# Oneaccount1/recommend-sys

Measured on NVIDIA B200. Metric: similarity_pairs_per_sec, higher is better.
Workload: dtype f64

## Files before the change

### recommend-sys_b200/csrc/api.cu

```cuda
#include <cstdlib>
#include <cstring>
#include <mutex>
#include <new>

#include "common.cuh"

static thread_local char g_err[512] = "";

void rs_set_error(const char *fmt, ...) {
    va_list ap;
    va_start(ap, fmt);
    vsnprintf(g_err, sizeof(g_err), fmt, ap);
    va_end(ap);
}

namespace {

int32_t enter(rs_knn *h) {
    if (!h) {
        rs_set_error("null handle");
        return RS_ERR_INVALID;
    }
    RS_CUDA(cudaSetDevice(h->device));
    return RS_OK;
}

struct Guard {
    std::unique_lock<std::recursive_mutex> lk;
    explicit Guard(rs_knn *h) { if (h) lk = std::unique_lock<std::recursive_mutex>(h->mu); }
};
#define RS_ENTER(h) Guard guard_(h); RS_TRY(enter(h))

void free_fit_state(rs_knn *h) {
    h->cur_chunk = 0;
    h->cur_off = 0;
    h->fitted = false;
    h->l_ptr = h->r_ptr = nullptr;
    h->l_col = h->r_col = nullptr;
    h->l_val = h->r_val = h->ld_val = nullptr;
    h->l_code = nullptr;
    h->means = h->stddevs = h->pmeans = h->left_bias = h->right_bias = nullptr;
    h->r_dev = nullptr;
    h->rd_col = nullptr;
    h->right_means = nullptr;
    h->cp = nullptr;
    h->l2r = nullptr;
    h->row_order = nullptr;
    h->row_heavy = nullptr;
    h->n_heavy = 0;
    h->n_pop = h->pop_ld = 0;
    h->pop_idx = h->pop_items = nullptr;
    h->pop_dense = nullptr;
    h->pop_blk = nullptr;
    h->w_ptr = nullptr;
    h->w_col = nullptr;
    h->w_dev = nullptr;
    h->row_all = nullptr;
    h->n_all_rows = 0;
    h->planes = nullptr;
    h->row_cnt = h->row_sum = nullptr;
    h->sims = nullptr;
    h->topk_idx = nullptr;
    h->topk_sim = nullptr;
    h->thr_key = nullptr;
    h->thr_id = nullptr;
    h->cand_cnt = nullptr;
    h->cand_id = nullptr;
    h->cand_sim = nullptr;
    h->row_flag = nullptr;
    h->d_flags = nullptr;
}

int32_t fold_profile(rs_knn *h) {
    RS_CUDA(cudaStreamSynchronize(h->stream));
    float ms = 0.f;
    if (h->prep_pending) {
        RS_CUDA(cudaEventElapsedTime(&ms, h->ev_a, h->ev_b));
        h->prof.prep_ms += ms;
        h->prep_pending = false;
    }
    if (h->sim_pending) {
        RS_CUDA(cudaEventElapsedTime(&ms, h->ev_b, h->ev_c));
        h->prof.sim_kernel_ms += ms;
        h->sim_pending = false;
    }
    if (h->pred_pending) {
        RS_CUDA(cudaEventElapsedTime(&ms, h->ev_d, h->ev_e));
        h->prof.predict_kernel_ms += ms;
        h->pred_pending = false;
    }
    return RS_OK;
}

bool tensor_eligible(const rs_knn *h) {
    if (h->rating_class != RS_CLASS_INT8) return false;
    if (h->p.sim == RS_SIM_COSINE || h->p.sim == RS_SIM_MSD || h->p.sim == RS_SIM_SLOPE_ONE) return true;
    if (h->p.sim == RS_SIM_PEARSON && h->p.pearson_mode == RS_PEARSON_SUMS) return true;
    return false;
}

bool tensor_faster(const rs_knn *h) {
    const double n = (double)h->n_left, rows = (double)(h->row_end - h->row_begin);
    const bool full = h->row_begin == 0 && h->row_end == h->n_left;
    const double g = h->p.sim == RS_SIM_COSINE ? 3.0 : h->p.sim == RS_SIM_MSD ? 4.0 : 6.0;
    const double pairs = full ? n * (n - 1.0) / 2.0 : rows * n;
    const double t_tensor = pairs * 2.0 * g * (double)h->n_right / 2.0e15 + 1e-4;
    const double triples = full ? h->triples : 2.0 * h->triples * (rows / n);
    const double t_stream = triples / 6.0e10 + 1e-4;
    return t_tensor <= t_stream;
}

struct IpcMap { int device; unsigned char handle[64]; void *base; };
std::mutex g_ipc_mu;
std::vector<IpcMap> g_ipc;

int32_t ipc_open_cached(int device, const unsigned char *hb, void **base) {
    std::lock_guard<std::mutex> lk(g_ipc_mu);
    for (const auto &m : g_ipc)
        if (m.device == device && !std::memcmp(m.handle, hb, 64)) { *base = m.base; return RS_OK; }
    cudaIpcMemHandle_t mh;
    std::memcpy(&mh, hb, 64);
    RS_CUDA(cudaIpcOpenMemHandle(base, mh, cudaIpcMemLazyEnablePeerAccess));
    IpcMap m;
    m.device = device;
    std::memcpy(m.handle, hb, 64);
    m.base = *base;
    g_ipc.push_back(m);
    return RS_OK;
}

int32_t init_handle(rs_knn *h) {
    RS_CUDA(cudaSetDevice(h->device));
    RS_CUDA(cudaStreamCreateWithFlags(&h->own_stream, cudaStreamNonBlocking));
    RS_CUDA(cudaStreamCreateWithFlags(&h->aux_stream, cudaStreamNonBlocking));
    RS_CUDA(cudaEventCreateWithFlags(&h->ev_in, cudaEventDisableTiming));
    RS_CUDA(cudaEventCreateWithFlags(&h->ev_fork, cudaEventDisableTiming));
    RS_CUDA(cudaEventCreateWithFlags(&h->ev_join, cudaEventDisableTiming));
    h->stream = h->own_stream;
    RS_CUDA(cudaEventCreate(&h->ev_a));
    RS_CUDA(cudaEventCreate(&h->ev_b));
    RS_CUDA(cudaEventCreate(&h->ev_c));
    RS_CUDA(cudaEventCreate(&h->ev_d));
    RS_CUDA(cudaEventCreate(&h->ev_e));
    return RS_OK;
}

}

extern "C" {

const char *rs_last_error(void) { return g_err; }
int32_t rs_knn_abi_version(void) { return 1; }

int32_t rs_knn_device_count(void) {
    int n = 0;
    if (cudaGetDeviceCount(&n) != cudaSuccess) {
        (void)cudaGetLastError();
        return 0;
    }
    return n;
}

int32_t rs_knn_params_default(rs_knn_params *p) {
    if (!p) return RS_ERR_INVALID;
    std::memset(p, 0, sizeof(*p));
    p->sim = RS_SIM_MSD;
    p->knn_type = RS_KNN_BASIC;
    p->k = 40;
    p->min_k = 1;
    p->device = -1;
    p->pearson_mode = RS_PEARSON_EXACT;
    p->sim_path = RS_PATH_AUTO;
    p->store = RS_STORE_MATRIX;
    p->topk = 40;
    return RS_OK;
}

int32_t rs_knn_create(const rs_knn_params *p, rs_knn **out) {
    if (!p || !out) {
        rs_set_error("rs_knn_create: null argument");
        return RS_ERR_INVALID;
    }
    if (p->sim < RS_SIM_COSINE || p->sim > RS_SIM_SLOPE_ONE || p->knn_type < RS_KNN_BASIC ||
        p->knn_type > RS_KNN_BASELINE || p->k < 1 || p->min_k < 0) {
        rs_set_error("rs_knn_create: invalid sim/knn_type/k/min_k");
        return RS_ERR_INVALID;
    }
    int ndev = 0;
    cudaError_t e = cudaGetDeviceCount(&ndev);
    if (e != cudaSuccess || ndev == 0) {
        (void)cudaGetLastError();
        rs_set_error("no CUDA device available (%s); this library has no CPU fallback",
                     e == cudaSuccess ? "0 devices" : cudaGetErrorString(e));
        return RS_ERR_CUDA;
    }
    int dev = p->device;
    if (dev < 0) RS_CUDA(cudaGetDevice(&dev));
    if (dev >= ndev) {
        rs_set_error("device %d out of range (%d devices)", dev, ndev);
        return RS_ERR_INVALID;
    }
    int cc_major = 0, cc_minor = 0;
    RS_CUDA(cudaDeviceGetAttribute(&cc_major, cudaDevAttrComputeCapabilityMajor, dev));
    RS_CUDA(cudaDeviceGetAttribute(&cc_minor, cudaDevAttrComputeCapabilityMinor, dev));
    if (cc_major != 10) {
        rs_set_error("device %d is sm_%d%d; this library is built for sm_100a (B200) only", dev, cc_major,
                     cc_minor);
        return RS_ERR_UNSUPPORTED;
    }
    rs_knn *h = new (std::nothrow) rs_knn();
    if (!h) return RS_ERR_OOM;
    h->p = *p;
    h->device = dev;
    const int32_t rc = init_handle(h);
    if (rc != RS_OK) {
        rs_knn_destroy(h);
        return rc;
    }
    *out = h;
    return RS_OK;
}

int32_t rs_knn_destroy(rs_knn *h) {
    if (!h) return RS_OK;
    cudaSetDevice(h->device);
    if (h->stream) cudaStreamSynchronize(h->stream);
    free_fit_state(h);
    for (auto &c : h->chunks) rs_cached_free(h->device, c.p, c.bytes);
    h->chunks.clear();
    if (h->tile_buf) cudaFree(h->tile_buf);
    if (h->band_buf) cudaFree(h->band_buf);
    if (h->ovf) rs_cached_free(h->device, h->ovf, h->ovf_bytes);
    for (size_t i = 0; i < h->scratch.size(); i++) rs_cached_free(h->device, h->scratch[i], h->scratch_bytes[i]);
    if (h->ev_a) cudaEventDestroy(h->ev_a);
    if (h->ev_b) cudaEventDestroy(h->ev_b);
    if (h->ev_c) cudaEventDestroy(h->ev_c);
    if (h->ev_d) cudaEventDestroy(h->ev_d);
    if (h->ev_e) cudaEventDestroy(h->ev_e);
    if (h->own_stream) cudaStreamDestroy(h->own_stream);
    if (h->aux_stream) cudaStreamDestroy(h->aux_stream);
    if (h->ev_in) cudaEventDestroy(h->ev_in);
    if (h->ev_fork) cudaEventDestroy(h->ev_fork);
    if (h->ev_join) cudaEventDestroy(h->ev_join);
    delete h;
    return RS_OK;
}

int32_t rs_knn_set_stream(rs_knn *h, void *cuda_stream, int32_t use_own) {
    RS_ENTER(h);
    RS_CUDA(cudaStreamSynchronize(h->stream));
    h->stream = use_own ? h->own_stream : reinterpret_cast<cudaStream_t>(cuda_stream);
    return RS_OK;
}

int32_t rs_knn_synchronize(rs_knn *h) {
    RS_ENTER(h);
    RS_CUDA(cudaStreamSynchronize(h->stream));
    return RS_OK;
}

int32_t rs_knn_fit_device(rs_knn *h, const int32_t *d_left, const int32_t *d_right, const double *d_rating,
                          int64_t nnz, int32_t n_left, int32_t n_right, double global_mean,
                          const double *d_left_bias, const double *d_right_bias, double global_bias) {
    RS_ENTER(h);
    if (!d_left || !d_right || !d_rating || nnz <= 0 || n_left <= 0 || n_right <= 0) {
        rs_set_error("rs_knn_fit: empty or null input (nnz=%lld n_left=%d n_right=%d)", (long long)nnz, n_left,
                     n_right);
        return RS_ERR_INVALID;
    }
    if (h->p.knn_type == RS_KNN_BASELINE && !d_left_bias) {
        rs_set_error("rs_knn_fit: RS_KNN_BASELINE needs left_bias (core/knn.go:179-187)");
        return RS_ERR_INVALID;
    }
    if (h->p.sim == RS_SIM_PEARSON_BASELINE && (!d_left_bias || !d_right_bias)) {
        rs_set_error("rs_knn_fit: RS_SIM_PEARSON_BASELINE needs both bias vectors");
        return RS_ERR_INVALID;
    }
    RS_TRY(fold_profile(h));
    free_fit_state(h);
    h->nnz = nnz;
    h->n_left = n_left;
    h->n_right = n_right;
    h->global_mean = global_mean;
    h->global_bias = global_bias;
    h->row_begin = h->p.row_begin;
    h->row_end = h->p.row_end;
    if (h->row_begin == 0 && h->row_end == 0) h->row_end = n_left;
    if (h->row_begin < 0 || h->row_end > n_left || h->row_begin > h->row_end) {
        rs_set_error("row shard [%lld,%lld) outside [0,%d)", (long long)h->row_begin, (long long)h->row_end, n_left);
        return RS_ERR_INVALID;
    }
    const int64_t rows = h->row_end - h->row_begin;
    if (h->p.shard_count < 0 || (h->p.shard_count >= 1 && (h->p.shard_index < 0 || h->p.shard_index >= h->p.shard_count))) {
        rs_set_error("shard_index %d outside [0, shard_count=%d)", h->p.shard_index, h->p.shard_count);
        return RS_ERR_INVALID;
    }
    if (h->p.shard_count >= 1 && rows != n_left) {
        rs_set_error("shard_count >= 1 and row_begin/row_end are two different sharding schemes: use one");
        return RS_ERR_INVALID;
    }
    h->cyc_R = (h->p.store == RS_STORE_MATRIX && h->p.shard_count >= 2) ? h->p.shard_count : 0;
    h->cyc_r = h->cyc_R ? h->p.shard_index : 0;
    h->peers_ready = false;
    if (h->cyc_R > RS_MAX_PEERS) {
        rs_set_error("at most %d cyclic row shards", RS_MAX_PEERS);
        return RS_ERR_UNSUPPORTED;
    }
    if (h->cyc_R && h->p.sim == RS_SIM_SLOPE_ONE) {
        rs_set_error("RS_SIM_SLOPE_ONE does not support cyclic row shards (use row_begin/row_end)");
        return RS_ERR_UNSUPPORTED;
    }
    h->rows_local = h->cyc_R ? rs_cyc_rows(n_left, h->cyc_R, h->cyc_r) : rows;

    RS_CUDA(cudaEventRecord(h->ev_a, h->stream));
    int32_t rc = rs_prep_build(h, d_left, d_right, d_rating, d_left_bias, d_right_bias);
    if (rc != RS_OK) { free_fit_state(h); return rc; }

    int path = h->p.sim_path;
    if (const char *force = getenv("RS_KNN_FORCE_PATH")) {
        if (!strcmp(force, "stream")) path = RS_PATH_STREAM;
        else if (!strcmp(force, "tensor")) path = RS_PATH_TENSOR;
    }
    if (h->p.sim == RS_SIM_SLOPE_ONE) {
        if (!tensor_eligible(h) || path == RS_PATH_STREAM) {
            rs_set_error("RS_SIM_SLOPE_ONE needs integer ratings in [-11,11] (tensor path)");
            free_fit_state(h);
            return RS_ERR_UNSUPPORTED;
        }
        path = RS_PATH_TENSOR;
    }
    if (h->cyc_R) {
        if (path == RS_PATH_TENSOR) {
            rs_set_error("cyclic row shards run the stream path; shard the tensor path with row_begin/row_end");
            free_fit_state(h);
            return RS_ERR_UNSUPPORTED;
        }
        path = RS_PATH_STREAM;
    }
    if (path == RS_PATH_AUTO) path = tensor_eligible(h) && tensor_faster(h) ? RS_PATH_TENSOR : RS_PATH_STREAM;
    if (path == RS_PATH_TENSOR && !tensor_eligible(h)) {
        rs_set_error("tensor path needs integer ratings in [-11,11] and Cosine/MSD (or Pearson in SUMS mode)");
        free_fit_state(h);
        return RS_ERR_UNSUPPORTED;
    }
    h->prof.sim_path_used = path;
    h->prof.corated_triples = h->triples;
    rc = (path == RS_PATH_TENSOR) ? rs_prep_planes(h) : rs_prep_rt(h);
    if (rc != RS_OK) { free_fit_state(h); return rc; }

    h->ld_s = ((int64_t)n_left + 15) / 16 * 16;
    if (h->p.store == RS_STORE_MATRIX) {
        rc = rs_alloc(h, &h->sims, (size_t)h->rows_local * (size_t)h->ld_s);
        if (rc != RS_OK) { free_fit_state(h); return rc; }
        RS_CUDA(cudaEventRecord(h->ev_b, h->stream));
        rc = (path == RS_PATH_TENSOR) ? rs_sim_tensor_launch(h, nullptr, 0, 0) : rs_sim_stream_launch(h);
        if (rc != RS_OK) { free_fit_state(h); return rc; }
        RS_CUDA(cudaEventRecord(h->ev_c, h->stream));
        if (path == RS_PATH_STREAM) {
            rc = rs_symmetrize_launch(h);
            if (rc != RS_OK) { free_fit_state(h); return rc; }
        }
    } else if (h->p.shard_count >= 1 && path == RS_PATH_TENSOR && rs_tensor_topk_fused(h)) {
        const int32_t k = h->p.topk > 0 ? h->p.topk : h->p.k;
        const int64_t n = n_left;
        h->cand_cap = 1792;
        if (const char *e = getenv("RS_KNN_TOPK_CAP")) h->cand_cap = atoi(e);
        if (k > 256 || h->cand_cap + k > 2048 || h->cand_cap < 1) {
            rs_set_error("fused top-k: k <= 256 and candidate capacity + k <= 2048 (k=%d cap=%d)", k, h->cand_cap);
            free_fit_state(h);
            return RS_ERR_UNSUPPORTED;
        }
        RS_TRY(rs_alloc(h, &h->topk_idx, (size_t)n * k));
        RS_TRY(rs_alloc(h, &h->topk_sim, (size_t)n * k));
        RS_TRY(rs_alloc(h, &h->thr_key, (size_t)n));
        RS_TRY(rs_alloc(h, &h->thr_id, (size_t)n));
        RS_TRY(rs_alloc(h, &h->cand_cnt, (size_t)n));
        RS_TRY(rs_alloc(h, &h->row_flag, (size_t)n));
        RS_TRY(rs_alloc(h, &h->cand_id, (size_t)n * h->cand_cap));
        RS_TRY(rs_alloc(h, &h->cand_sim, (size_t)n * h->cand_cap));
        h->topk_rows = n;
        RS_CUDA(cudaMemsetAsync(h->topk_idx, 0xFF, (size_t)n * k * 4, h->stream));
        RS_CUDA(cudaMemsetAsync(h->topk_sim, 0xFF, (size_t)n * k * 8, h->stream));
        RS_CUDA(cudaMemsetAsync(h->thr_key, 0, (size_t)n * 8, h->stream));
        RS_CUDA(cudaMemsetAsync(h->thr_id, 0xFF, (size_t)n * 4, h->stream));
        RS_CUDA(cudaMemsetAsync(h->cand_cnt, 0, (size_t)n * 4, h->stream));
        RS_CUDA(cudaMemsetAsync(h->row_flag, 0, (size_t)n * 4, h->stream));
        int32_t *d_over = h->d_flags + 14;
        RS_CUDA(cudaEventRecord(h->ev_b, h->stream));
        const int n_waves = rs_tensor_band_count(h);
        for (int w = 0; w < n_waves && rc == RS_OK; w++) {
            int rerun = 0;
            for (;;) {
                RS_CUDA(cudaMemsetAsync(d_over, 0, 4, h->stream));
                rc = rs_sim_tensor_band_launch(h, w);
                if (rc == RS_OK) rc = rs_topk_compact_launch(h, k, d_over, rerun);
                if (rc != RS_OK) break;
                int32_t over = 0;
                RS_CUDA(cudaMemcpyAsync(&over, d_over, 4, cudaMemcpyDeviceToHost, h->stream));
                RS_CUDA(cudaStreamSynchronize(h->stream));
                if (rerun) rc = rs_topk_mask_launch(h, k, 1);
                if (over == 0 || rc != RS_OK) break;
                rc = rs_topk_mask_launch(h, k, 0);
                rerun = 1;
            }
        }
        if (rc != RS_OK) { free_fit_state(h); return rc; }
        RS_CUDA(cudaEventRecord(h->ev_c, h->stream));
    } else if (h->p.shard_count >= 1) {
        const int32_t k = h->p.topk > 0 ? h->p.topk : h->p.k;
        const int64_t n = n_left;
        int64_t m = (int64_t)(6ll << 30) / (h->ld_s * 8);
        if (h->p.shard_count > 1) {
            int64_t want = (n + 4ll * h->p.shard_count - 1) / (4ll * h->p.shard_count);
            want = (want + 255) / 256 * 256;
            if (want < 1024) want = 1024;
            if (want < m) m = want;
        }
        if (const char *e = getenv("RS_KNN_SLAB_ROWS")) m = atoll(e);
        if (m < 256) m = 256;
        m = m / 256 * 256;
        if (m > n) m = (n + 15) / 16 * 16;
        const int64_t ld_t = m;
        double *tbuf = nullptr;
        RS_TRY(rs_alloc(h, &h->sims, (size_t)m * (size_t)h->ld_s));
        RS_TRY(rs_alloc(h, &tbuf, (size_t)n * (size_t)ld_t));
        RS_TRY(rs_alloc(h, &h->topk_idx, (size_t)n * k));
        RS_TRY(rs_alloc(h, &h->topk_sim, (size_t)n * k));
        h->topk_rows = n;
        RS_CUDA(cudaMemsetAsync(h->topk_idx, 0xFF, (size_t)n * k * 4, h->stream));
        RS_CUDA(cudaMemsetAsync(h->topk_sim, 0xFF, (size_t)n * k * 8, h->stream));
        RS_CUDA(cudaEventRecord(h->ev_b, h->stream));
        const int64_t n_slabs = (n + m - 1) / m;
        h->force_sym = true;
        for (int64_t sl = 0; sl < n_slabs; sl++) {
            const int64_t round = sl / h->p.shard_count, posn = sl % h->p.shard_count;
            const int64_t owner = (round & 1) ? h->p.shard_count - 1 - posn : posn;
            if (owner != h->p.shard_index) continue;
            const int64_t r0 = sl * m, r1 = r0 + m < n ? r0 + m : n;
            h->row_begin = r0;
            h->row_end = r1;
            h->col_begin = r0;
            if (path == RS_PATH_STREAM) {
                rc = cudaMemsetAsync(h->sims, 0xFF, (size_t)(r1 - r0) * (size_t)h->ld_s * 8, h->stream) == cudaSuccess
                         ? RS_OK : RS_ERR_CUDA;
                if (rc == RS_OK) rc = rs_sim_stream_launch(h);
            } else {
                rc = rs_sim_tensor_launch(h, nullptr, 0, 0);
            }
            if (rc == RS_OK) rc = rs_topk_slab_launch(h, r0, (int32_t)(r1 - r0), tbuf, ld_t, k);
            if (rc != RS_OK) break;
        }
        h->force_sym = false;
        h->col_begin = 0;
        h->row_begin = 0;
        h->row_end = n;
        if (rc != RS_OK) { free_fit_state(h); return rc; }
        RS_CUDA(cudaEventRecord(h->ev_c, h->stream));
    } else {
        const int32_t k = h->p.topk > 0 ? h->p.topk : h->p.k;
        int64_t slab = (int64_t)(2ull << 30) / ((int64_t)h->ld_s * 8);
        if (slab < 128) slab = 128;
        slab = slab / 128 * 128;
        if (slab > rows) slab = rows;
        RS_TRY(rs_alloc(h, &h->sims, (size_t)slab * (size_t)h->ld_s));
        RS_TRY(rs_alloc(h, &h->topk_idx, (size_t)rows * k));
        RS_TRY(rs_alloc(h, &h->topk_sim, (size_t)rows * k));
        h->topk_rows = rows;
        RS_CUDA(cudaEventRecord(h->ev_b, h->stream));
        const int64_t rb = h->row_begin, re = h->row_end;
        for (int64_t r0 = rb; r0 < re; r0 += slab) {
            h->row_begin = r0;
            h->row_end = r0 + slab < re ? r0 + slab : re;
            rc = (path == RS_PATH_TENSOR) ? rs_sim_tensor_launch(h, nullptr, 0, 0) : rs_sim_stream_launch(h);
            if (rc == RS_OK && path == RS_PATH_STREAM) rc = rs_symmetrize_launch(h);
            if (rc == RS_OK)
                rc = rs_topk_launch(h, k, h->topk_idx + (r0 - rb) * k, h->topk_sim + (r0 - rb) * k);
            if (rc != RS_OK) break;
        }
        h->row_begin = rb;
        h->row_end = re;
        if (rc != RS_OK) { free_fit_state(h); return rc; }
        RS_CUDA(cudaEventRecord(h->ev_c, h->stream));
    }
    h->prep_pending = true;
    h->sim_pending = true;
    h->fitted = true;
    return RS_OK;
}

int32_t rs_scratch_get(rs_knn *h, int slot, size_t bytes, void **out) {
    if (h->scratch.size() <= (size_t)slot) {
        h->scratch.resize(slot + 1, nullptr);
        h->scratch_bytes.resize(slot + 1, 0);
    }
    if (h->scratch_bytes[slot] < bytes) {
        if (h->scratch[slot]) {
            RS_CUDA(cudaStreamSynchronize(h->stream));
            rs_cached_free(h->device, h->scratch[slot], h->scratch_bytes[slot]);
        }
        h->scratch[slot] = nullptr;
        h->scratch_bytes[slot] = 0;
        size_t want = bytes + bytes / 4 + 256, got = 0;
        RS_TRY(rs_cached_malloc(h->device, &h->scratch[slot], want, &got));
        h->scratch_bytes[slot] = got;
    }
    *out = h->scratch[slot];
    return RS_OK;
}

int32_t rs_knn_fit(rs_knn *h, const int32_t *left, const int32_t *right, const double *rating, int64_t nnz,
                   int32_t n_left, int32_t n_right, double global_mean, const double *left_bias,
                   const double *right_bias, double global_bias) {
    RS_ENTER(h);
    if (!left || !right || !rating || nnz <= 0 || n_left <= 0 || n_right <= 0) {
        rs_set_error("rs_knn_fit: empty or null input (nnz=%lld n_left=%d n_right=%d)", (long long)nnz, n_left,
                     n_right);
        return RS_ERR_INVALID;
    }
    void *d_left, *d_right, *d_rating, *d_lb = nullptr, *d_rb = nullptr;
    RS_TRY(rs_scratch_get(h, 7, (size_t)nnz * 4, &d_left));
    RS_TRY(rs_scratch_get(h, 8, (size_t)nnz * 4, &d_right));
    RS_TRY(rs_scratch_get(h, 9, (size_t)nnz * 8, &d_rating));
    RS_CUDA(cudaMemcpyAsync(d_left, left, (size_t)nnz * 4, cudaMemcpyHostToDevice, h->stream));
    RS_CUDA(cudaMemcpyAsync(d_right, right, (size_t)nnz * 4, cudaMemcpyHostToDevice, h->stream));
    RS_CUDA(cudaMemcpyAsync(d_rating, rating, (size_t)nnz * 8, cudaMemcpyHostToDevice, h->stream));
    if (left_bias) {
        RS_TRY(rs_scratch_get(h, 10, (size_t)n_left * 8, &d_lb));
        RS_CUDA(cudaMemcpyAsync(d_lb, left_bias, (size_t)n_left * 8, cudaMemcpyHostToDevice, h->stream));
    }
    if (right_bias) {
        RS_TRY(rs_scratch_get(h, 11, (size_t)n_right * 8, &d_rb));
        RS_CUDA(cudaMemcpyAsync(d_rb, right_bias, (size_t)n_right * 8, cudaMemcpyHostToDevice, h->stream));
    }
    RS_CUDA(cudaEventRecord(h->ev_in, h->stream));
    RS_TRY(rs_knn_fit_device(h, (const int32_t *)d_left, (const int32_t *)d_right, (const double *)d_rating, nnz,
                             n_left, n_right, global_mean, (const double *)d_lb, (const double *)d_rb,
                             global_bias));
    cudaError_t e = cudaEventSynchronize(h->ev_in);
    if (e != cudaSuccess) {
        rs_set_error("rs_knn_fit: %s", cudaGetErrorString(e));
        h->fitted = false;
        return RS_ERR_CUDA;
    }
    return RS_OK;
}

static int32_t require_matrix(rs_knn *h, const char *who) {
    if (!h->fitted) {
        rs_set_error("%s: Fit has not been called", who);
        return RS_ERR_INVALID;
    }
    if (h->p.store != RS_STORE_MATRIX) {
        rs_set_error("%s needs RS_STORE_MATRIX (the handle keeps top-k lists only)", who);
        return RS_ERR_INVALID;
    }
    if (h->cyc_R > 1 && !h->peers_ready) {
        rs_set_error("%s: cyclic row shards hold one triangle of their rows until rs_knn_mirror has run", who);
        return RS_ERR_INVALID;
    }
    return RS_OK;
}

int32_t rs_knn_predict_batch_device(rs_knn *h, const int32_t *d_left, const int32_t *d_right, int64_t n,
                                    double *d_out) {
    RS_ENTER(h);
    RS_TRY(require_matrix(h, "rs_knn_predict_batch"));
    if (n == 0) return RS_OK;
    if (!d_left || !d_right || !d_out || n < 0) {
        rs_set_error("rs_knn_predict_batch: null argument");
        return RS_ERR_INVALID;
    }
    if (h->pred_pending) RS_TRY(fold_profile(h));
    RS_CUDA(cudaEventRecord(h->ev_d, h->stream));
    if (h->p.sim == RS_SIM_SLOPE_ONE) RS_TRY(rs_slope_predict_launch(h, d_left, d_right, n, d_out));
    else RS_TRY(rs_predict_launch(h, d_left, d_right, n, d_out, nullptr, nullptr, nullptr, 0));
    RS_CUDA(cudaEventRecord(h->ev_e, h->stream));
    h->pred_pending = true;
    return RS_OK;
}

int32_t rs_knn_predict_batch_sharded_device(rs_knn *h, const int32_t *d_left, const int32_t *d_right, int64_t n,
                                            double *d_out) {
    RS_ENTER(h);
    RS_TRY(require_matrix(h, "rs_knn_predict_batch_sharded"));
    if (h->cyc_R < 2) {
        rs_set_error("rs_knn_predict_batch_sharded: the handle is not a cyclic row shard");
        return RS_ERR_INVALID;
    }
    if (n == 0) return RS_OK;
    if (!d_left || !d_right || !d_out || n < 0) {
        rs_set_error("rs_knn_predict_batch_sharded: null argument");
        return RS_ERR_INVALID;
    }
    if (h->pred_pending) RS_TRY(fold_profile(h));
    RS_CUDA(cudaEventRecord(h->ev_d, h->stream));
    RS_TRY(rs_predict_launch(h, d_left, d_right, n, d_out, nullptr, nullptr, nullptr, 0, 1));
    RS_CUDA(cudaEventRecord(h->ev_e, h->stream));
    h->pred_pending = true;
    return RS_OK;
}

int32_t rs_knn_predict_batch(rs_knn *h, const int32_t *left, const int32_t *right, int64_t n, double *out) {
    RS_ENTER(h);
    RS_TRY(require_matrix(h, "rs_knn_predict_batch"));
    if (n == 0) return RS_OK;
    if (!left || !right || !out || n < 0) {
        rs_set_error("rs_knn_predict_batch: null argument");
        return RS_ERR_INVALID;
    }
    void *dl, *dr, *dout;
    RS_TRY(rs_scratch_get(h, 0, (size_t)n * 4, &dl));
    RS_TRY(rs_scratch_get(h, 1, (size_t)n * 4, &dr));
    RS_TRY(rs_scratch_get(h, 2, (size_t)n * 8, &dout));
    RS_CUDA(cudaMemcpyAsync(dl, left, (size_t)n * 4, cudaMemcpyHostToDevice, h->stream));
    RS_CUDA(cudaMemcpyAsync(dr, right, (size_t)n * 4, cudaMemcpyHostToDevice, h->stream));
    RS_TRY(rs_knn_predict_batch_device(h, (const int32_t *)dl, (const int32_t *)dr, n, (double *)dout));
    RS_CUDA(cudaMemcpyAsync(out, dout, (size_t)n * 8, cudaMemcpyDeviceToHost, h->stream));
    RS_CUDA(cudaStreamSynchronize(h->stream));
    return RS_OK;
}

int32_t rs_knn_predict_neighbors(rs_knn *h, int32_t left, int32_t right, int32_t cap, int32_t *ids, double *sims,
                                 int32_t *n_out) {
    RS_ENTER(h);
    RS_TRY(require_matrix(h, "rs_knn_predict_neighbors"));
    if (!ids || !sims || !n_out || cap < 1) {
        rs_set_error("rs_knn_predict_neighbors: null argument");
        return RS_ERR_INVALID;
    }
    void *dl, *dr, *dout, *dids, *dsims, *dcnt;
    RS_TRY(rs_scratch_get(h, 0, 4, &dl));
    RS_TRY(rs_scratch_get(h, 1, 4, &dr));
    RS_TRY(rs_scratch_get(h, 2, 8, &dout));
    RS_TRY(rs_scratch_get(h, 3, (size_t)cap * 4, &dids));
    RS_TRY(rs_scratch_get(h, 4, (size_t)cap * 8, &dsims));
    RS_TRY(rs_scratch_get(h, 5, 4, &dcnt));
    RS_CUDA(cudaMemcpyAsync(dl, &left, 4, cudaMemcpyHostToDevice, h->stream));
    RS_CUDA(cudaMemcpyAsync(dr, &right, 4, cudaMemcpyHostToDevice, h->stream));
    RS_CUDA(cudaMemsetAsync(dcnt, 0, 4, h->stream));
    RS_TRY(rs_predict_launch(h, (const int32_t *)dl, (const int32_t *)dr, 1, (double *)dout, (int32_t *)dids,
                             (double *)dsims, (int32_t *)dcnt, cap));
    RS_TRY(rs_nb_cells_launch(h, (const int32_t *)dl, (const int32_t *)dids, (const int32_t *)dcnt, (double *)dsims));
    int32_t cnt = 0;
    RS_CUDA(cudaMemcpyAsync(&cnt, dcnt, 4, cudaMemcpyDeviceToHost, h->stream));
    RS_CUDA(cudaStreamSynchronize(h->stream));
    if (cnt > 0) {
        RS_CUDA(cudaMemcpy(ids, dids, (size_t)cnt * 4, cudaMemcpyDeviceToHost));
        RS_CUDA(cudaMemcpy(sims, dsims, (size_t)cnt * 8, cudaMemcpyDeviceToHost));
    }
    *n_out = cnt;
    return RS_OK;
}

int32_t rs_knn_sims_rows(rs_knn *h, int64_t row0, int64_t nrows, double *out) {
    RS_ENTER(h);
    RS_TRY(require_matrix(h, "rs_knn_sims_rows"));
    if (!out || nrows < 0 || row0 < h->row_begin || row0 + nrows > h->row_end) {
        rs_set_error("rs_knn_sims_rows: rows [%lld,%lld) outside the shard [%lld,%lld)", (long long)row0,
                     (long long)(row0 + nrows), (long long)h->row_begin, (long long)h->row_end);
        return RS_ERR_INVALID;
    }
    if (nrows == 0) return RS_OK;
    int64_t local0 = row0 - h->row_begin;
    if (h->cyc_R > 1) {
        if (!rs_cyc_owns(row0, h->cyc_R, h->cyc_r) || row0 / RS_CYC_B != (row0 + nrows - 1) / RS_CYC_B) {
            rs_set_error("rs_knn_sims_rows: rows [%lld,%lld) are not inside one %d-row block of shard %d of %d",
                         (long long)row0, (long long)(row0 + nrows), RS_CYC_B, h->cyc_r, h->cyc_R);
            return RS_ERR_INVALID;
        }
        local0 = rs_cyc_local(row0, h->cyc_R);
    }
    RS_CUDA(cudaMemcpy2DAsync(out, (size_t)h->n_left * 8, h->sims + local0 * h->ld_s,
                              (size_t)h->ld_s * 8, (size_t)h->n_left * 8, (size_t)nrows, cudaMemcpyDeviceToHost,
                              h->stream));
    RS_CUDA(cudaStreamSynchronize(h->stream));
    return RS_OK;
}

int32_t rs_knn_topk_device(rs_knn *h, int32_t k, int32_t *d_idx, double *d_sim) {
    RS_ENTER(h);
    if (!h->fitted || !d_idx || !d_sim) {
        rs_set_error("rs_knn_topk: not fitted or null argument");
        return RS_ERR_INVALID;
    }
    const int64_t rows = h->p.store == RS_STORE_TOPK ? h->topk_rows : h->rows_local;
    if (h->p.store == RS_STORE_MATRIX) RS_TRY(require_matrix(h, "rs_knn_topk"));
    if (h->p.store == RS_STORE_TOPK) {
        const int32_t kk = h->p.topk > 0 ? h->p.topk : h->p.k;
        if (k != kk) {
            rs_set_error("rs_knn_topk: handle holds top-%d lists, asked for %d", kk, k);
            return RS_ERR_INVALID;
        }
        RS_CUDA(cudaMemcpyAsync(d_idx, h->topk_idx, (size_t)rows * k * 4, cudaMemcpyDeviceToDevice, h->stream));
        RS_CUDA(cudaMemcpyAsync(d_sim, h->topk_sim, (size_t)rows * k * 8, cudaMemcpyDeviceToDevice, h->stream));
        return RS_OK;
    }
    return rs_topk_launch(h, k, d_idx, d_sim);
}

int32_t rs_knn_topk(rs_knn *h, int32_t k, int32_t *idx, double *sim) {
    RS_ENTER(h);
    if (!h->fitted || !idx || !sim || k < 1) {
        rs_set_error("rs_knn_topk: not fitted or bad argument");
        return RS_ERR_INVALID;
    }
    const int64_t rows = h->p.store == RS_STORE_TOPK ? h->topk_rows : h->rows_local;
    void *di, *ds;
    RS_TRY(rs_scratch_get(h, 3, (size_t)rows * k * 4, &di));
    RS_TRY(rs_scratch_get(h, 4, (size_t)rows * k * 8, &ds));
    RS_TRY(rs_knn_topk_device(h, k, (int32_t *)di, (double *)ds));
    RS_CUDA(cudaMemcpyAsync(idx, di, (size_t)rows * k * 4, cudaMemcpyDeviceToHost, h->stream));
    RS_CUDA(cudaMemcpyAsync(sim, ds, (size_t)rows * k * 8, cudaMemcpyDeviceToHost, h->stream));
    RS_CUDA(cudaStreamSynchronize(h->stream));
    return RS_OK;
}

int32_t rs_knn_cosums(rs_knn *h, int64_t row0, int64_t nrows, int32_t *out) {
    RS_ENTER(h);
    if (!h->fitted || !out || nrows < 0 || row0 < 0 || row0 + nrows > h->n_left) {
        rs_set_error("rs_knn_cosums: not fitted or bad argument");
        return RS_ERR_INVALID;
    }
    if (h->rating_class != RS_CLASS_INT8) {
        rs_set_error("rs_knn_cosums: integer co-rating sums need integer ratings in [-11,11]");
        return RS_ERR_UNSUPPORTED;
    }
    if (nrows == 0) return RS_OK;
    if (!h->planes) RS_TRY(rs_prep_planes(h));
    void *d;
    const size_t bytes = (size_t)nrows * (size_t)h->n_left * 6 * 4;
    RS_TRY(rs_scratch_get(h, 6, bytes, &d));
    RS_TRY(rs_sim_tensor_launch(h, (int32_t *)d, row0, nrows));
    RS_CUDA(cudaMemcpyAsync(out, d, bytes, cudaMemcpyDeviceToHost, h->stream));
    RS_CUDA(cudaStreamSynchronize(h->stream));
    return RS_OK;
}

static int32_t copy_vec(rs_knn *h, const double *d, double *out, const char *who) {
    RS_ENTER(h);
    if (!h->fitted || !out || !d) {
        rs_set_error("%s: not fitted or null argument", who);
        return RS_ERR_INVALID;
    }
    RS_CUDA(cudaMemcpyAsync(out, d, (size_t)h->n_left * 8, cudaMemcpyDeviceToHost, h->aux_stream));
    RS_CUDA(cudaStreamSynchronize(h->aux_stream));
    return RS_OK;
}

int32_t rs_knn_means(rs_knn *h, double *out) { return copy_vec(h, h ? h->means : nullptr, out, "rs_knn_means"); }
int32_t rs_knn_stddevs(rs_knn *h, double *out) {
    if (h && h->p.knn_type != RS_KNN_ZSCORE) {
        rs_set_error("rs_knn_stddevs: only the z-score KNN keeps StdDevs (core/knn.go:167)");
        return RS_ERR_INVALID;
    }
    return copy_vec(h, h ? h->stddevs : nullptr, out, "rs_knn_stddevs");
}

int32_t rs_knn_set_k(rs_knn *h, int32_t k, int32_t min_k) {
    RS_ENTER(h);
    if (k < 1 || min_k < 0) {
        rs_set_error("rs_knn_set_k: k >= 1 and min_k >= 0 required");
        return RS_ERR_INVALID;
    }
    h->p.k = k;
    h->p.min_k = min_k;
    return RS_OK;
}

int32_t rs_knn_peer_export(rs_knn *h, unsigned char *handle64, int64_t *offset) {
    RS_ENTER(h);
    if (!h->fitted || h->cyc_R < 2 || !handle64 || !offset) {
        rs_set_error("rs_knn_peer_export: the handle is not a fitted cyclic row shard");
        return RS_ERR_INVALID;
    }
    for (const auto &c : h->chunks) {
        const char *s0 = reinterpret_cast<const char *>(h->sims);
        if (s0 >= c.p && s0 < c.p + c.bytes) {
            cudaIpcMemHandle_t mh;
            RS_CUDA(cudaIpcGetMemHandle(&mh, c.p));
            static_assert(sizeof(mh) == 64, "cudaIpcMemHandle_t is 64 bytes");
            std::memcpy(handle64, &mh, 64);
            *offset = (int64_t)(s0 - c.p);
            return RS_OK;
        }
    }
    rs_set_error("rs_knn_peer_export: the matrix is not in the handle's arena");
    return RS_ERR_INVALID;
}

int32_t rs_knn_peer_import(rs_knn *h, int32_t n_peers, const unsigned char *handles, const int64_t *offsets) {
    RS_ENTER(h);
    if (!h->fitted || h->cyc_R < 2 || n_peers != h->cyc_R || !handles || !offsets) {
        rs_set_error("rs_knn_peer_import: needs a fitted cyclic row shard and one (handle, offset) per shard");
        return RS_ERR_INVALID;
    }
    for (int q = 0; q < n_peers; q++) {
        if (q == h->cyc_r) { h->peer_sims[q] = h->sims; continue; }
        const unsigned char *hb = handles + (size_t)q * 64;
        void *base = nullptr;
        RS_TRY(ipc_open_cached(h->device, hb, &base));
        h->peer_sims[q] = reinterpret_cast<const double *>(static_cast<const char *>(base) + offsets[q]);
    }
    return RS_OK;
}

int32_t rs_knn_peer_import_local(rs_knn *h, int32_t n_peers, rs_knn *const *peers) {
    RS_ENTER(h);
    if (!h->fitted || h->cyc_R < 2 || n_peers != h->cyc_R || !peers) {
        rs_set_error("rs_knn_peer_import_local: needs a fitted cyclic row shard and one handle per shard");
        return RS_ERR_INVALID;
    }
    for (int q = 0; q < n_peers; q++) {
        const rs_knn *o = peers[q];
        if (!o || !o->fitted || o->cyc_R != h->cyc_R || o->cyc_r != q || o->n_left != h->n_left || o->ld_s != h->ld_s) {
            rs_set_error("rs_knn_peer_import_local: peer %d is not shard %d of the same Fit", q, q);
            return RS_ERR_INVALID;
        }
        if (o->device != h->device) {
            int can = 0;
            RS_CUDA(cudaDeviceCanAccessPeer(&can, h->device, o->device));
            if (!can) {
                rs_set_error("device %d cannot access device %d", h->device, o->device);
                return RS_ERR_UNSUPPORTED;
            }
            cudaError_t e = cudaDeviceEnablePeerAccess(o->device, 0);
            if (e != cudaSuccess && e != cudaErrorPeerAccessAlreadyEnabled) RS_CUDA(e);
            (void)cudaGetLastError();
        }
        h->peer_sims[q] = o->sims;
    }
    return RS_OK;
}

int32_t rs_knn_mirror(rs_knn *h) {
    RS_ENTER(h);
    if (!h->fitted || h->cyc_R < 2) {
        rs_set_error("rs_knn_mirror: the handle is not a fitted cyclic row shard");
        return RS_ERR_INVALID;
    }
    for (int q = 0; q < h->cyc_R; q++)
        if (q != h->cyc_r && !h->peer_sims[q]) {
            rs_set_error("rs_knn_mirror: shard %d has not been attached (rs_knn_peer_import)", q);
            return RS_ERR_INVALID;
        }
    RS_TRY(rs_mirror_launch(h));
    h->peers_ready = true;
    return RS_OK;
}

int32_t rs_knn_profile_get(rs_knn *h, rs_knn_profile *out) {
    RS_ENTER(h);
    if (!out) return RS_ERR_INVALID;
    RS_TRY(fold_profile(h));
    *out = h->prof;
    return RS_OK;
}

namespace {
struct HostBlock { void *p; size_t bytes; bool used; };
std::mutex g_host_mu;
std::vector<HostBlock> g_host;
}

int32_t rs_knn_host_alloc(size_t bytes, void **out) {
    if (!out) { rs_set_error("rs_knn_host_alloc: null argument"); return RS_ERR_INVALID; }
    if (bytes == 0) bytes = 1;
    std::lock_guard<std::mutex> lk(g_host_mu);
    HostBlock *best = nullptr;
    for (auto &b : g_host)
        if (!b.used && b.bytes >= bytes && b.bytes <= 2 * bytes + 4096 && (!best || b.bytes < best->bytes)) best = &b;
    if (best) { best->used = true; *out = best->p; return RS_OK; }
    void *p = nullptr;
    RS_CUDA(cudaHostAlloc(&p, bytes, cudaHostAllocPortable));
    g_host.push_back({p, bytes, true});
    *out = p;
    return RS_OK;
}

int32_t rs_knn_host_free(void *p) {
    if (!p) return RS_OK;
    std::lock_guard<std::mutex> lk(g_host_mu);
    for (auto &b : g_host)
        if (b.p == p && b.used) { b.used = false; return RS_OK; }
    rs_set_error("rs_knn_host_free: not a block of rs_knn_host_alloc");
    return RS_ERR_INVALID;
}

int32_t rs_knn_trim_cache(void) {
    rs_cache_trim();
    {
        std::lock_guard<std::mutex> lk(g_host_mu);
        size_t kept = 0;
        for (auto &b : g_host) {
            if (b.used) g_host[kept++] = b;
            else cudaFreeHost(b.p);
        }
        g_host.resize(kept);
    }
    std::lock_guard<std::mutex> lk(g_ipc_mu);
    int cur = 0;
    cudaGetDevice(&cur);
    for (const auto &m : g_ipc) {
        cudaSetDevice(m.device);
        cudaIpcCloseMemHandle(m.base);
    }
    g_ipc.clear();
    cudaSetDevice(cur);
    return RS_OK;
}

int32_t rs_knn_profile_reset(rs_knn *h) {
    RS_ENTER(h);
    RS_TRY(fold_profile(h));
    int32_t path = h->prof.sim_path_used;
    h->prof = rs_knn_profile{};
    h->prof.sim_path_used = path;
    h->prof.corated_triples = h->triples;
    return RS_OK;
}

}
```

### recommend-sys_b200/csrc/common.cuh

```cuda
#pragma once

#include <cuda_runtime.h>

#include <cstdarg>
#include <cstdint>
#include <cstdio>
#include <mutex>
#include <vector>

#include "rs_knn.h"

void rs_set_error(const char *fmt, ...);

#define RS_CUDA(expr)                                                                       \
    do {                                                                                    \
        cudaError_t e_ = (expr);                                                            \
        if (e_ != cudaSuccess) {                                                            \
            rs_set_error("%s: %s (%s:%d)", #expr, cudaGetErrorString(e_), __FILE__, __LINE__); \
            return (e_ == cudaErrorMemoryAllocation) ? RS_ERR_OOM : RS_ERR_CUDA;            \
        }                                                                                   \
    } while (0)

#define RS_TRY(expr)              \
    do {                          \
        int32_t rc_ = (expr);     \
        if (rc_ != RS_OK) return rc_; \
    } while (0)

enum { RS_CLASS_INT8 = 0, RS_CLASS_TABLE = 1 };
constexpr int RS_INT8_BIAS = 12;

constexpr int RS_STREAM_WARPS = 8;

constexpr int RS_TC_BM = 128;
constexpr int RS_TC_BN = 64;
constexpr int RS_TC_BK = 128;
constexpr int RS_TC_KBLK = 256;

constexpr int RS_CYC_B = 32;
constexpr int RS_MAX_PEERS = 16;
__host__ __device__ inline int64_t rs_cyc_local(int64_t i, int count) {
    return (i / ((int64_t)RS_CYC_B * count)) * RS_CYC_B + i % RS_CYC_B;
}
__host__ __device__ inline bool rs_cyc_owns(int64_t i, int count, int index) {
    return (i / RS_CYC_B) % count == index;
}
inline int64_t rs_cyc_rows(int64_t n, int count, int index) {
    const int64_t nblk = (n + RS_CYC_B - 1) / RS_CYC_B;
    int64_t rows = 0;
    for (int64_t b = index; b < nblk; b += count) rows += (b + 1) * RS_CYC_B <= n ? RS_CYC_B : n - b * RS_CYC_B;
    return rows;
}

struct rs_knn {
    std::recursive_mutex mu;
    rs_knn_params p{};
    int device = 0;
    cudaStream_t own_stream = nullptr;
    cudaStream_t stream = nullptr;
    cudaStream_t aux_stream = nullptr;
    cudaEvent_t ev_in = nullptr;
    cudaEvent_t ev_fork = nullptr, ev_join = nullptr;
    cudaEvent_t ev_a = nullptr, ev_b = nullptr, ev_c = nullptr, ev_d = nullptr, ev_e = nullptr;
    rs_knn_profile prof{};
    bool sim_pending = false, pred_pending = false, prep_pending = false;

    bool fitted = false;
    int32_t n_left = 0, n_right = 0;
    int64_t nnz = 0;
    int64_t row_begin = 0, row_end = 0;
    int64_t col_begin = 0;
    bool force_sym = false;
    int64_t topk_rows = 0;
    int32_t cyc_R = 0, cyc_r = 0;
    int64_t rows_local = 0;
    int64_t n_work_rows = 0;
    const double *peer_sims[RS_MAX_PEERS] = {nullptr};
    bool peers_ready = false;
    double global_mean = 0.0, global_bias = 0.0;
    int rating_class = RS_CLASS_INT8;

    struct Chunk { char *p; size_t bytes; };
    std::vector<Chunk> chunks;
    size_t cur_chunk = 0, cur_off = 0;
    void *tile_buf = nullptr;
    size_t tile_buf_bytes = 0;
    int64_t tile_key[5] = {-1, -1, -1, -1, -1};
    int32_t tile_count = 0;
    void *band_buf = nullptr;
    size_t band_buf_bytes = 0;
    int64_t band_key[4] = {-1, -1, -1, -1};
    std::vector<int64_t> band_off;
    unsigned long long *thr_key = nullptr;
    int32_t *thr_id = nullptr;
    int32_t *cand_cnt = nullptr;
    int32_t *cand_id = nullptr;
    double *cand_sim = nullptr;
    int32_t cand_cap = 0;
    int32_t *row_flag = nullptr;

    int64_t *l_ptr = nullptr;
    int32_t *l_col = nullptr;
    double *l_val = nullptr;
    uint8_t *l_code = nullptr;
    double *ld_val = nullptr;
    int64_t *r_ptr = nullptr;
    int32_t *r_col = nullptr;
    double *r_val = nullptr;

    double *means = nullptr;
    double *stddevs = nullptr;
    double *pmeans = nullptr;
    double *left_bias = nullptr;
    int32_t *row_cnt = nullptr;
    int32_t *row_sum = nullptr;
    int64_t max_row_cnt = 0;
    int32_t max_right_len = 0;
    double triples = 0.0;
    double *right_bias = nullptr;
    int32_t *rd_col = nullptr;
    double *right_means = nullptr;

    double *r_dev = nullptr;
    int32_t *cp = nullptr;
    int32_t n_chunks = 0;
    int32_t stream_jc = 256;
    bool stream_lower = false;
    double inc_upper = 0.0, inc_lower = 0.0;
    int64_t *l2r = nullptr;
    int32_t *perm_lr = nullptr, *perm_rl = nullptr, *perm_tmp = nullptr;
    int32_t *row_order = nullptr;
    int32_t *row_heavy = nullptr;
    int32_t n_heavy = 0;
    int32_t n_pop = 0, pop_ld = 0;
    bool pop_u8 = false;
    int32_t *pop_idx = nullptr;
    int32_t *pop_items = nullptr;
    uint8_t *pop_blk = nullptr;
    void *pop_dense = nullptr;
    int64_t *w_ptr = nullptr;
    int32_t *w_col = nullptr;
    double *w_dev = nullptr;
    int32_t *row_all = nullptr;
    int64_t n_all_rows = 0;
    int8_t *planes = nullptr;
    int64_t tc_npad = 0, tc_kpad = 0;

    double *sims = nullptr;
    int64_t ld_s = 0;
    int32_t *topk_idx = nullptr;
    double *topk_sim = nullptr;

    int32_t *d_flags = nullptr;
    void *ovf = nullptr;
    size_t ovf_bytes = 0;
    std::vector<void *> scratch;
    std::vector<size_t> scratch_bytes;
};

int32_t rs_cached_malloc(int device, void **out, size_t bytes, size_t *got);
void rs_cached_free(int device, void *p, size_t bytes);
void rs_cache_trim(void);

extern "C" int32_t rs_scratch_get(rs_knn *h, int slot, size_t bytes, void **out);

int32_t rs_prep_build(rs_knn *h, const int32_t *d_left, const int32_t *d_right, const double *d_rating,
                      const double *d_left_bias, const double *d_right_bias);
int32_t rs_dev_alloc(rs_knn *h, void **out, size_t bytes);
template <typename T>
inline int32_t rs_alloc(rs_knn *h, T **out, size_t count) {
    return rs_dev_alloc(h, reinterpret_cast<void **>(out), count * sizeof(T));
}
int32_t rs_prep_rt(rs_knn *h);
int32_t rs_prep_planes(rs_knn *h);

int32_t rs_sim_stream_launch(rs_knn *h);
int32_t rs_symmetrize_launch(rs_knn *h);
int32_t rs_mirror_launch(rs_knn *h);

int32_t rs_sim_tensor_launch(rs_knn *h, int32_t *d_cosums, int64_t cos_row0, int64_t cos_nrows);
int32_t rs_tensor_band_count(const rs_knn *h);
int32_t rs_sim_tensor_band_launch(rs_knn *h, int32_t wave);
bool rs_tensor_topk_fused(const rs_knn *h);

int32_t rs_predict_launch(rs_knn *h, const int32_t *d_left, const int32_t *d_right, int64_t n, double *d_out,
                          int32_t *d_nb_ids, double *d_nb_sims, int32_t *d_nb_count, int32_t nb_cap, int32_t foreign_zero = 0);
int32_t rs_nb_cells_launch(rs_knn *h, const int32_t *d_left, const int32_t *d_nb_ids, const int32_t *d_nb_count,
                           double *d_nb_sims);
int32_t rs_topk_launch(rs_knn *h, int32_t k, int32_t *d_idx, double *d_sim);
int32_t rs_slope_predict_launch(rs_knn *h, const int32_t *d_left, const int32_t *d_right, int64_t n, double *d_out);
int32_t rs_topk_slab_launch(rs_knn *h, int64_t g0, int32_t m, double *tbuf, int64_t ld_t, int32_t k);
int32_t rs_topk_compact_launch(rs_knn *h, int32_t k, int32_t *d_overflow, int rerun);
int32_t rs_topk_mask_launch(rs_knn *h, int32_t k, int restore);

__host__ __device__ inline uint64_t rs_sim_key(double s) {
    s = s + 0.0;
#ifdef __CUDA_ARCH__
    uint64_t b = (uint64_t)__double_as_longlong(s);
#else
    uint64_t b;
    __builtin_memcpy(&b, &s, 8);
#endif
    return (b & 0x8000000000000000ull) ? ~b : (b | 0x8000000000000000ull);
}
__host__ __device__ inline double rs_key_sim(uint64_t k) {
    uint64_t b = (k & 0x8000000000000000ull) ? (k & 0x7fffffffffffffffull) : ~k;
#ifdef __CUDA_ARCH__
    return __longlong_as_double((long long)b);
#else
    double s;
    __builtin_memcpy(&s, &b, 8);
    return s;
#endif
}
```

### recommend-sys_b200/csrc/prep.cu

```cuda
#include <cub/cub.cuh>

#include <cstdlib>
#include <cstring>

#include "common.cuh"

int32_t rs_dev_alloc(rs_knn *h, void **out, size_t bytes) {
    bytes = (bytes + 255) & ~(size_t)255;
    if (bytes == 0) bytes = 256;
    while (h->cur_chunk < h->chunks.size()) {
        rs_knn::Chunk &c = h->chunks[h->cur_chunk];
        if (h->cur_off + bytes <= c.bytes) {
            *out = c.p + h->cur_off;
            h->cur_off += bytes;
            return RS_OK;
        }
        h->cur_chunk++;
        h->cur_off = 0;
    }
    const size_t min_chunk = (size_t)64 << 20;
    const size_t want = bytes > min_chunk ? bytes : min_chunk;
    void *p = nullptr;
    size_t got = 0;
    RS_TRY(rs_cached_malloc(h->device, &p, want, &got));
    h->chunks.push_back({(char *)p, got});
    h->cur_chunk = h->chunks.size() - 1;
    h->cur_off = bytes;
    *out = p;
    return RS_OK;
}

namespace {

constexpr int T = 256;
inline unsigned blocks_for(int64_t n, int t = T) { return (unsigned)((n + t - 1) / t); }

enum { FLAG_BAD_ID = 1, FLAG_NOT_INT8 = 2, FLAG_DUP = 4, FLAG_NAN = 8 };

__global__ void iota_validate_kernel(const int32_t *__restrict__ left, const int32_t *__restrict__ right,
                                     const double *__restrict__ rating, int64_t nnz, int32_t n_left,
                                     int32_t n_right, int32_t *__restrict__ idx, int32_t *__restrict__ flags) {
    int64_t i = (int64_t)blockIdx.x * blockDim.x + threadIdx.x;
    if (i >= nnz) return;
    idx[i] = (int32_t)i;
    int32_t l = left[i], r = right[i];
    int f = 0;
    if (l < 0 || l >= n_left || r < 0 || r >= n_right) f |= FLAG_BAD_ID;
    double v = rating[i];
    if (v != v) f |= FLAG_NAN;
    if (!(v == rint(v) && fabs(v) <= 11.0)) f |= FLAG_NOT_INT8;
    if (f) atomicOr(flags, f);
}

__global__ void ptr_from_sorted_kernel(const int32_t *__restrict__ keys, int64_t nnz, int32_t n_rows,
                                       int64_t *__restrict__ ptr) {
    const int64_t i = (int64_t)blockIdx.x * blockDim.x + threadIdx.x;
    if (i > nnz) return;
    const int32_t cur = i < nnz ? keys[i] : n_rows;
    const int32_t prev = i > 0 ? keys[i - 1] : -1;
    for (int32_t k = prev + 1; k <= cur; k++) ptr[k] = i;
}

__global__ void gather_keys_kernel(const int32_t *__restrict__ src, const int32_t *__restrict__ perm, int64_t n,
                                   int32_t *__restrict__ out) {
    int64_t i = (int64_t)blockIdx.x * blockDim.x + threadIdx.x;
    if (i < n) out[i] = src[perm[i]];
}

__global__ void gather_csr_kernel(const int32_t *__restrict__ perm, const int32_t *__restrict__ minor,
                                  const double *__restrict__ rating, int64_t nnz, int32_t *__restrict__ col,
                                  double *__restrict__ val) {
    int64_t i = (int64_t)blockIdx.x * blockDim.x + threadIdx.x;
    if (i >= nnz) return;
    int32_t p = perm[i];
    col[i] = minor[p];
    val[i] = rating[p];
}

__global__ void dup_check_kernel(const int32_t *__restrict__ row, const int32_t *__restrict__ col, int64_t nnz,
                                 int32_t *__restrict__ flags) {
    int64_t i = (int64_t)blockIdx.x * blockDim.x + threadIdx.x;
    if (i == 0 || i >= nnz) return;
    if (row[i] == row[i - 1] && col[i] == col[i - 1]) atomicOr(flags, FLAG_DUP);
}

__global__ void gather_val_kernel(const int32_t *__restrict__ perm, const double *__restrict__ rating, int64_t nnz,
                                  double *__restrict__ val) {
    int64_t i = (int64_t)blockIdx.x * blockDim.x + threadIdx.x;
    if (i < nnz) val[i] = rating[perm[i]];
}

__global__ void code_int8_kernel(const double *__restrict__ val, int64_t nnz, uint8_t *__restrict__ code) {
    int64_t i = (int64_t)blockIdx.x * blockDim.x + threadIdx.x;
    if (i < nnz) code[i] = (uint8_t)((int)val[i] + RS_INT8_BIAS);
}

__global__ void row_isum_kernel(const int64_t *__restrict__ l_ptr, const uint8_t *__restrict__ l_code,
                                int32_t n_left, int32_t *__restrict__ row_cnt, int32_t *__restrict__ row_sum) {
    int32_t row = (int32_t)(((int64_t)blockIdx.x * blockDim.x + threadIdx.x) >> 5);
    int lane = threadIdx.x & 31;
    if (row >= n_left) return;
    int s = 0;
    for (int64_t x = l_ptr[row] + lane; x < l_ptr[row + 1]; x += 32) s += (int)l_code[x] - RS_INT8_BIAS;
    for (int o = 16; o > 0; o >>= 1) s += __shfl_xor_sync(0xffffffffu, s, o);
    if (lane == 0) {
        row_cnt[row] = (int32_t)(l_ptr[row + 1] - l_ptr[row]);
        row_sum[row] = s;
    }
}

__device__ __forceinline__ double ordered_sum(const double *__restrict__ v, int64_t b, int64_t e, int lane,
                                              double mean, bool squared_dev) {
    double sum = 0.0;
    for (int64_t base = b; base < e; base += 32) {
        double x = (base + lane < e) ? v[base + lane] : 0.0;
        if (squared_dev) x = (x - mean) * (x - mean);
        const int lim = (e - base) < 32 ? (int)(e - base) : 32;
        for (int q = 0; q < lim; q++) sum += __shfl_sync(0xffffffffu, x, q);
    }
    return sum;
}

__global__ void row_stats_ordered_kernel(const int64_t *__restrict__ l_ptr, const double *__restrict__ ld_val,
                                         const double *__restrict__ l_val, int32_t n_left, int want_mean,
                                         int want_std, double *__restrict__ means, double *__restrict__ stddevs,
                                         double *__restrict__ pmeans) {
    const int32_t i = (int32_t)(((int64_t)blockIdx.x * blockDim.x + threadIdx.x) >> 5);
    const int lane = threadIdx.x & 31;
    if (i >= n_left) return;
    const int64_t b = l_ptr[i], e = l_ptr[i + 1];
    const double count = (double)(e - b);
    double mean = means[i];
    if (want_mean) {
        mean = ordered_sum(ld_val, b, e, lane, 0.0, false) / count;
        const double pm = ordered_sum(l_val, b, e, lane, 0.0, false) / count;
        if (lane == 0) { means[i] = mean; pmeans[i] = pm; }
    }
    if (want_std) {
        const double s2 = ordered_sum(ld_val, b, e, lane, mean, true);
        if (lane == 0) stddevs[i] = sqrt(s2 / count) + 1e-5;
    }
}

__global__ void means_from_isum_kernel(const int32_t *__restrict__ row_cnt, const int32_t *__restrict__ row_sum,
                                       int32_t n_left, double *__restrict__ means, double *__restrict__ pmeans) {
    const int32_t i = blockIdx.x * blockDim.x + threadIdx.x;
    if (i >= n_left) return;
    const double m = (double)row_sum[i] / (double)row_cnt[i];
    means[i] = m;
    pmeans[i] = m;
}

__global__ void build_rdev_kernel(const int64_t *__restrict__ r_ptr, const int32_t *__restrict__ r_col,
                                  const double *__restrict__ r_val, int32_t n_right, int sim,
                                  const double *__restrict__ pmeans, const double *__restrict__ left_bias,
                                  const double *__restrict__ right_bias, double global_bias,
                                  double *__restrict__ r_dev) {
    const int32_t c = (int32_t)(((int64_t)blockIdx.x * blockDim.x + threadIdx.x) >> 5);
    const int lane = threadIdx.x & 31;
    if (c >= n_right) return;
    for (int64_t x = r_ptr[c] + lane; x < r_ptr[c + 1]; x += 32) {
        const int32_t j = r_col[x];
        const double y = r_val[x];
        double t;
        if (sim == RS_SIM_PEARSON) t = y - pmeans[j];
        else if (sim == RS_SIM_PEARSON_BASELINE) { const double base = global_bias + left_bias[j]; const double bb = base + right_bias[c]; t = y - bb; }
        else t = y;
        r_dev[x] = t;
    }
}

__global__ void row_len_kernel(const int64_t *__restrict__ l_ptr, int32_t n_left, int32_t *__restrict__ len,
                               int32_t *__restrict__ ids) {
    const int32_t i = blockIdx.x * blockDim.x + threadIdx.x;
    if (i >= n_left) return;
    len[i] = (int32_t)(l_ptr[i + 1] - l_ptr[i]);
    ids[i] = i;
}

__global__ void build_cp_kernel(const int64_t *__restrict__ r_ptr, const int32_t *__restrict__ r_col,
                                int32_t n_right, int32_t q0, int32_t n_q, int32_t jc, int32_t *__restrict__ cp) {
    const int32_t c = (int32_t)(((int64_t)blockIdx.x * blockDim.x + threadIdx.x) >> 5);
    const int lane = threadIdx.x & 31;
    if (c >= n_right) return;
    const int64_t b = r_ptr[c], e = r_ptr[c + 1];
    int32_t *out = cp + (int64_t)c * (n_q + 1);
    auto rel = [&](int32_t col) {
        const int32_t q = col / jc - q0;
        return q < 0 ? -1 : (q >= n_q ? n_q : q);
    };
    for (int64_t x0 = b; x0 <= e; x0 += 32) {
        const int64_t x = x0 + lane;
        if (x > e) continue;
        const int32_t cur = x < e ? rel(r_col[x]) : n_q;
        const int32_t prev = x > b ? rel(r_col[x - 1]) : -1;
        for (int32_t q = prev + 1; q <= cur; q++) out[q] = (int32_t)(x - b);
    }
}

__global__ void invert_perm_kernel(const int32_t *__restrict__ perm, int64_t n, int32_t *__restrict__ inv) {
    const int64_t x = (int64_t)blockIdx.x * blockDim.x + threadIdx.x;
    if (x < n) inv[perm[x]] = (int32_t)x;
}
__global__ void compose_l2r_kernel(const int32_t *__restrict__ perm_lr, const int32_t *__restrict__ inv_rl, int64_t n,
                                   int64_t *__restrict__ l2r) {
    const int64_t e = (int64_t)blockIdx.x * blockDim.x + threadIdx.x;
    if (e < n) l2r[e] = inv_rl[perm_lr[e]];
}

__global__ void pop_count_kernel(const int32_t *__restrict__ len_sorted, int32_t n, int64_t min_len, int32_t cap,
                                 int32_t *__restrict__ out) {
    int32_t lo = 0, hi = n;
    while (lo < hi) {
        const int32_t mid = (lo + hi) >> 1;
        if ((int64_t)len_sorted[mid] >= min_len) lo = mid + 1; else hi = mid;
    }
    *out = lo < cap ? lo : cap;
}
__global__ void pop_index_kernel(const int32_t *__restrict__ sorted, int32_t n_pop, int32_t pop_ld,
                                 int32_t *__restrict__ pop_idx, int32_t *__restrict__ pop_items,
                                 uint8_t *__restrict__ pop_blk) {
    const int32_t p = blockIdx.x * blockDim.x + threadIdx.x;
    if (p >= pop_ld) return;
    if (p < n_pop) { const int32_t i = sorted[p]; pop_idx[i] = p; pop_items[p] = i; pop_blk[i >> 5] = 1; }
    else pop_items[p] = -1;
}
template <typename DT>
__global__ void pop_scatter_kernel(const int64_t *__restrict__ r_ptr, const int32_t *__restrict__ r_col,
                                   const double *__restrict__ r_val, const double *__restrict__ r_dev,
                                   int32_t n_right, const int32_t *__restrict__ pop_idx, int32_t pop_ld,
                                   DT *__restrict__ dense, int64_t *__restrict__ w_cnt) {
    const int32_t c = (int32_t)(((int64_t)blockIdx.x * blockDim.x + threadIdx.x) >> 5);
    const int lane = threadIdx.x & 31;
    if (c > n_right) return;
    if (c == n_right) { if (lane == 0) w_cnt[c] = 0; return; }
    int32_t light = 0;
    for (int64_t x = r_ptr[c] + lane; x < r_ptr[c + 1]; x += 32) {
        const int32_t p = pop_idx[r_col[x]];
        if (p < 0) { light++; continue; }
        if (sizeof(DT) == 1) dense[(int64_t)c * pop_ld + p] = (DT)((int)r_val[x] + RS_INT8_BIAS);
        else dense[(int64_t)c * pop_ld + p] = (DT)r_dev[x];
    }
#pragma unroll
    for (int o = 16; o > 0; o >>= 1) light += __shfl_xor_sync(0xffffffffu, light, o);
    if (lane == 0) w_cnt[c] = light;
}
__global__ void pop_compact_kernel(const int64_t *__restrict__ r_ptr, const int32_t *__restrict__ r_col,
                                   const double *__restrict__ r_dev, int32_t n_right,
                                   const int32_t *__restrict__ pop_idx, const int64_t *__restrict__ w_ptr,
                                   int32_t *__restrict__ w_col, double *__restrict__ w_dev, int64_t *__restrict__ pos) {
    const int32_t c = (int32_t)(((int64_t)blockIdx.x * blockDim.x + threadIdx.x) >> 5);
    const int lane = threadIdx.x & 31;
    if (c >= n_right) return;
    const int64_t b = r_ptr[c], e = r_ptr[c + 1];
    int64_t out = w_ptr[c];
    for (int64_t x0 = b; x0 < e; x0 += 32) {
        const int64_t x = x0 + lane;
        int32_t j = -1;
        bool keep = false;
        if (x < e) { j = r_col[x]; keep = pop_idx[j] < 0; }
        const unsigned m = __ballot_sync(0xffffffffu, keep);
        if (x < e) {
            const int64_t o = out + __popc(m & ((1u << lane) - 1u));
            if (keep) { w_col[o] = j; w_dev[o] = r_dev[x]; pos[x] = o; }
            else pos[x] = -1;
        }
        out += __popc(m);
    }
}
__global__ void pop_remap_l2r_kernel(int64_t *__restrict__ l2r, const int64_t *__restrict__ pos, int64_t n) {
    const int64_t e = (int64_t)blockIdx.x * blockDim.x + threadIdx.x;
    if (e < n) l2r[e] = pos[l2r[e]];
}
struct PopLight {
    const int32_t *pop_idx;
    __host__ __device__ bool operator()(const int32_t &i) const { return pop_idx[i] < 0; }
};


__global__ void scatter_planes_kernel(const int64_t *__restrict__ l_ptr, const int32_t *__restrict__ l_col,
                                      const uint8_t *__restrict__ l_code, int32_t n_left, int64_t npad,
                                      int64_t kpad, int32_t kblk, int8_t *__restrict__ planes) {
    int32_t row = (int32_t)(((int64_t)blockIdx.x * blockDim.x + threadIdx.x) >> 5);
    int lane = threadIdx.x & 31;
    if (row >= n_left) return;
    int64_t plane = npad * kpad;
    for (int64_t x = l_ptr[row] + lane; x < l_ptr[row + 1]; x += 32) {
        int v = (int)l_code[x] - RS_INT8_BIAS;
        const int32_t col = l_col[x];
        int64_t o = ((int64_t)(col / kblk) * npad + row) * kblk + (col % kblk);
        planes[o] = (int8_t)(v * v);
        planes[plane + o] = 1;
        planes[2 * plane + o] = (int8_t)v;
    }
}

struct CycOwned {
    int count, index;
    __host__ __device__ bool operator()(const int32_t &i) const { return rs_cyc_owns(i, count, index); }
};

struct SortTmp {
    void *p = nullptr;
    size_t bytes = 0;
};

int bits_for(int32_t n) {
    int b = 1;
    while ((1ll << b) < (long long)n) b++;
    return b;
}

}

#define RS_SORT_PAIRS(keys_in, keys_out, vals_in, vals_out, n, end_bit)                                      \
    do {                                                                                                     \
        size_t need_ = 0;                                                                                    \
        RS_CUDA(cub::DeviceRadixSort::SortPairs(nullptr, need_, keys_in, keys_out, vals_in, vals_out, (int)(n), \
                                                0, end_bit, st));                                            \
        if (need_ > tmp.bytes) {                                                                             \
            RS_TRY(rs_dev_alloc(h, &tmp.p, need_));                                                          \
            tmp.bytes = need_;                                                                               \
        }                                                                                                    \
        RS_CUDA(cub::DeviceRadixSort::SortPairs(tmp.p, tmp.bytes, keys_in, keys_out, vals_in, vals_out,      \
                                                (int)(n), 0, end_bit, st));                                  \
    } while (0)

__global__ void triples_kernel(const int64_t *__restrict__ r_ptr, int32_t nr, unsigned long long *out,
                               int32_t *max_len) {
    unsigned long long acc = 0;
    int32_t mx = 0;
    for (int64_t c = blockIdx.x * (int64_t)blockDim.x + threadIdx.x; c < nr; c += (int64_t)gridDim.x * blockDim.x) {
        const int32_t cnt = (int32_t)(r_ptr[c + 1] - r_ptr[c]);
        const unsigned long long n = (unsigned long long)cnt;
        acc += n * (n - (n ? 1 : 0)) / 2;
        mx = cnt > mx ? cnt : mx;
    }
#pragma unroll
    for (int o = 16; o > 0; o >>= 1) { const int32_t v = __shfl_xor_sync(0xffffffffu, mx, o); mx = v > mx ? v : mx; }
    if ((threadIdx.x & 31) == 0 && mx) atomicMax(max_len, mx);
#pragma unroll
    for (int o = 16; o > 0; o >>= 1) acc += __shfl_xor_sync(0xffffffffu, acc, o);
    if ((threadIdx.x & 31) == 0 && acc) atomicAdd(out, acc);
}

__global__ void incidence_kernel(const int64_t *__restrict__ l_ptr, int32_t nl, int32_t jc,
                                 unsigned long long *out) {
    unsigned long long up = 0, lo = 0;
    const long long q_all = (nl + jc - 1) / jc;
    for (int64_t i = blockIdx.x * (int64_t)blockDim.x + threadIdx.x; i < nl; i += (int64_t)gridDim.x * blockDim.x) {
        const unsigned long long d = (unsigned long long)(l_ptr[i + 1] - l_ptr[i]);
        const long long q = i / jc;
        up += d * (unsigned long long)(q_all - q);
        lo += d * (unsigned long long)(q + 1);
    }
#pragma unroll
    for (int o = 16; o > 0; o >>= 1) {
        up += __shfl_xor_sync(0xffffffffu, up, o);
        lo += __shfl_xor_sync(0xffffffffu, lo, o);
    }
    if ((threadIdx.x & 31) == 0) { atomicAdd(out, up); atomicAdd(out + 1, lo); }
}

__global__ void right_means_kernel(const int64_t *__restrict__ r_ptr, const double *__restrict__ r_val, int32_t nr,
                                   double *__restrict__ out) {
    const int32_t c = (int32_t)(((int64_t)blockIdx.x * blockDim.x + threadIdx.x) >> 5);
    const int lane = threadIdx.x & 31;
    if (c >= nr) return;
    double s = 0.0;
    for (int64_t x = r_ptr[c] + lane; x < r_ptr[c + 1]; x += 32) s += r_val[x];
#pragma unroll
    for (int o = 16; o > 0; o >>= 1) s += __shfl_xor_sync(0xffffffffu, s, o);
    if (lane == 0) out[c] = s / (double)(r_ptr[c + 1] - r_ptr[c]);
}

static int32_t rs_stream_jc(int32_t n_left) {
    int32_t jc = n_left < 8192 ? 128 : 256;
    if (const char *e = getenv("RS_KNN_STREAM_JC")) jc = atoi(e) == 128 ? 128 : 256;
    return jc;
}

int32_t rs_prep_build(rs_knn *h, const int32_t *d_left, const int32_t *d_right, const double *d_rating,
                      const double *d_left_bias, const double *d_right_bias) {
    cudaStream_t st = h->stream;
    const int64_t nnz = h->nnz;
    const int32_t nl = h->n_left, nr = h->n_right;
    if (nnz >= (1ll << 31)) {
        rs_set_error("nnz %lld exceeds the 2^31-1 entries supported", (long long)nnz);
        return RS_ERR_UNSUPPORTED;
    }
    SortTmp tmp;
    int32_t *idx, *keys_a, *keys_b, *perm_l, *perm_r, *perm_lr, *perm_rl;
    RS_TRY(rs_alloc(h, &idx, nnz));
    RS_TRY(rs_alloc(h, &keys_a, nnz));
    RS_TRY(rs_alloc(h, &keys_b, nnz));
    RS_TRY(rs_alloc(h, &perm_l, nnz));
    RS_TRY(rs_alloc(h, &perm_r, nnz));
    RS_TRY(rs_alloc(h, &perm_lr, nnz));
    RS_TRY(rs_alloc(h, &perm_rl, nnz));
    RS_TRY(rs_alloc(h, &h->d_flags, 16));
    RS_TRY(rs_alloc(h, &h->l_ptr, (size_t)nl + 1));
    RS_TRY(rs_alloc(h, &h->r_ptr, (size_t)nr + 1));
    RS_CUDA(cudaMemsetAsync(h->d_flags, 0, 64, st));

    iota_validate_kernel<<<blocks_for(nnz), T, 0, st>>>(d_left, d_right, d_rating, nnz, nl, nr, idx, h->d_flags);
    h->stream_jc = rs_stream_jc(nl);
    h->prof.total_launches += 1;
    int32_t flags = 0;
    RS_CUDA(cudaMemcpyAsync(&flags, h->d_flags, 4, cudaMemcpyDeviceToHost, st));
    RS_CUDA(cudaStreamSynchronize(st));
    if (flags & FLAG_BAD_ID) {
        rs_set_error("rating rows contain inner ids outside [0,n_left) x [0,n_right)");
        return RS_ERR_INVALID;
    }
    if (flags & FLAG_NAN) {
        rs_set_error("NaN ratings are not supported");
        return RS_ERR_UNSUPPORTED;
    }
    h->rating_class = (flags & FLAG_NOT_INT8) ? RS_CLASS_TABLE : RS_CLASS_INT8;

    const int lb = bits_for(nl), rb = bits_for(nr);
    const bool need_dataset_order = h->rating_class != RS_CLASS_INT8 || h->p.knn_type == RS_KNN_ZSCORE;
    if (need_dataset_order) RS_SORT_PAIRS(d_left, keys_a, idx, perm_l, nnz, lb);
    RS_SORT_PAIRS(d_right, keys_a, idx, perm_r, nnz, rb);
    ptr_from_sorted_kernel<<<blocks_for(nnz + 1), T, 0, st>>>(keys_a, nnz, nr, h->r_ptr);
    triples_kernel<<<148, T, 0, st>>>(h->r_ptr, nr, reinterpret_cast<unsigned long long *>(h->d_flags + 6), h->d_flags + 15);
    gather_keys_kernel<<<blocks_for(nnz), T, 0, st>>>(d_left, perm_r, nnz, keys_a);
    RS_SORT_PAIRS(keys_a, keys_b, perm_r, perm_lr, nnz, lb);
    ptr_from_sorted_kernel<<<blocks_for(nnz + 1), T, 0, st>>>(keys_b, nnz, nl, h->l_ptr);
    incidence_kernel<<<148, T, 0, st>>>(h->l_ptr, nl, h->stream_jc, reinterpret_cast<unsigned long long *>(h->d_flags + 8));
    h->prof.total_launches += 4;
    gather_keys_kernel<<<blocks_for(nnz), T, 0, st>>>(d_right, perm_lr, nnz, keys_a);
    RS_SORT_PAIRS(keys_a, keys_b, perm_lr, perm_rl, nnz, rb);
    h->prof.total_launches += 2;
    if (h->p.sim == RS_SIM_SLOPE_ONE) {
        RS_TRY(rs_alloc(h, &h->rd_col, nnz));
        gather_keys_kernel<<<blocks_for(nnz), T, 0, st>>>(d_left, perm_r, nnz, h->rd_col);
        h->prof.total_launches++;
    }
    h->perm_lr = perm_lr;
    h->perm_rl = perm_rl;
    h->perm_tmp = keys_b;

    RS_TRY(rs_alloc(h, &h->l_col, nnz));
    RS_TRY(rs_alloc(h, &h->l_val, nnz));
    RS_TRY(rs_alloc(h, &h->ld_val, nnz));
    RS_TRY(rs_alloc(h, &h->r_col, nnz));
    RS_TRY(rs_alloc(h, &h->r_val, nnz));
    gather_csr_kernel<<<blocks_for(nnz), T, 0, st>>>(perm_lr, d_right, d_rating, nnz, h->l_col, h->l_val);
    gather_csr_kernel<<<blocks_for(nnz), T, 0, st>>>(perm_rl, d_left, d_rating, nnz, h->r_col, h->r_val);
    dup_check_kernel<<<blocks_for(nnz), T, 0, st>>>(keys_b, h->r_col, nnz, h->d_flags);
    if (need_dataset_order) gather_val_kernel<<<blocks_for(nnz), T, 0, st>>>(perm_l, d_rating, nnz, h->ld_val);
    h->prof.total_launches += need_dataset_order ? 4 : 3;

    if (h->rating_class == RS_CLASS_INT8) {
        RS_TRY(rs_alloc(h, &h->l_code, nnz));
        code_int8_kernel<<<blocks_for(nnz), T, 0, st>>>(h->l_val, nnz, h->l_code);
        h->prof.total_launches += 1;
    }

    RS_TRY(rs_alloc(h, &h->means, (size_t)nl + 1));
    RS_TRY(rs_alloc(h, &h->stddevs, (size_t)nl + 1));
    RS_TRY(rs_alloc(h, &h->pmeans, (size_t)nl + 1));
    const int want_std = h->p.knn_type == RS_KNN_ZSCORE;
    if (h->rating_class == RS_CLASS_INT8) {
        RS_TRY(rs_alloc(h, &h->row_cnt, (size_t)nl + 1));
        RS_TRY(rs_alloc(h, &h->row_sum, (size_t)nl + 1));
        row_isum_kernel<<<blocks_for((int64_t)nl * 32), T, 0, st>>>(h->l_ptr, h->l_code, nl, h->row_cnt, h->row_sum);
        means_from_isum_kernel<<<blocks_for(nl), T, 0, st>>>(h->row_cnt, h->row_sum, nl, h->means, h->pmeans);
        h->prof.total_launches += 2;
    }
    if (h->rating_class != RS_CLASS_INT8 || want_std) {
        row_stats_ordered_kernel<<<blocks_for((int64_t)nl * 32), T, 0, st>>>(
            h->l_ptr, h->ld_val, h->l_val, nl, h->rating_class != RS_CLASS_INT8, want_std, h->means, h->stddevs,
            h->pmeans);
        h->prof.total_launches++;
    }

    if (h->p.sim == RS_SIM_SLOPE_ONE) {
        RS_TRY(rs_alloc(h, &h->right_means, (size_t)nr + 1));
        right_means_kernel<<<blocks_for((int64_t)nr * 32), T, 0, st>>>(h->r_ptr, h->r_val, nr, h->right_means);
        h->prof.total_launches++;
    }
    if (d_left_bias) {
        RS_TRY(rs_alloc(h, &h->left_bias, (size_t)nl + 1));
        RS_CUDA(cudaMemcpyAsync(h->left_bias, d_left_bias, (size_t)nl * 8, cudaMemcpyDeviceToDevice, st));
    }
    if (d_right_bias) {
        RS_TRY(rs_alloc(h, &h->right_bias, (size_t)nr + 1));
        RS_CUDA(cudaMemcpyAsync(h->right_bias, d_right_bias, (size_t)nr * 8, cudaMemcpyDeviceToDevice, st));
    }

    int32_t fl8[16] = {0};
    RS_CUDA(cudaMemcpyAsync(fl8, h->d_flags, 64, cudaMemcpyDeviceToHost, st));
    RS_CUDA(cudaStreamSynchronize(st));
    flags = fl8[0];
    { unsigned long long t; memcpy(&t, fl8 + 6, 8); h->triples = (double)t; }
    h->max_right_len = fl8[15];
    { unsigned long long t[2]; memcpy(t, fl8 + 8, 16); h->inc_upper = (double)t[0]; h->inc_lower = (double)t[1]; }
    h->stream_lower = h->inc_lower < h->inc_upper;
    if (const char *e = getenv("RS_KNN_STREAM_TRI")) h->stream_lower = !strcmp(e, "lower");
    if (flags & FLAG_DUP) {
        rs_set_error("duplicate (left,right) rating pairs are not supported (the reference's merge-join "
                     "double-counts them)");
        return RS_ERR_DUPLICATE;
    }
    RS_CUDA(cudaGetLastError());
    return RS_OK;
}

struct HeavyPred {
    const int64_t *l_ptr;
    int64_t min_len;
    bool negate;
    __host__ __device__ bool operator()(const int32_t &i) const { return ((l_ptr[i + 1] - l_ptr[i]) >= min_len) != negate; }
};

static int32_t split_heavy_rows(rs_knn *h, int32_t *order, int64_t n_rows, bool allow) {
    cudaStream_t st = h->stream;
    int64_t min_len = h->cyc_R > 1 ? 8192 : -1;
    if (const char *e = getenv("RS_KNN_HEAVY_MIN")) min_len = atoll(e);
    h->n_heavy = 0;
    h->row_heavy = nullptr;
    h->row_order = order;
    h->n_work_rows = n_rows;
    if (n_rows <= 0 || !allow || min_len < 0 || h->stream_jc != 256) return RS_OK;
    int32_t *rest, *d_num;
    RS_TRY(rs_alloc(h, &h->row_heavy, (size_t)n_rows));
    RS_TRY(rs_alloc(h, &rest, (size_t)n_rows));
    RS_TRY(rs_alloc(h, &d_num, 4));
    HeavyPred yes{h->l_ptr, min_len, false}, no{h->l_ptr, min_len, true};
    size_t need = 0;
    RS_CUDA(cub::DeviceSelect::If(nullptr, need, order, h->row_heavy, d_num, (int)n_rows, yes, st));
    void *tmp;
    RS_TRY(rs_dev_alloc(h, &tmp, need + 256));
    RS_CUDA(cub::DeviceSelect::If(tmp, need, order, h->row_heavy, d_num, (int)n_rows, yes, st));
    RS_CUDA(cub::DeviceSelect::If(tmp, need, order, rest, d_num + 1, (int)n_rows, no, st));
    int32_t cnt = 0;
    RS_CUDA(cudaMemcpyAsync(&cnt, d_num, 4, cudaMemcpyDeviceToHost, st));
    RS_CUDA(cudaStreamSynchronize(st));
    h->n_heavy = cnt;
    h->row_order = rest;
    h->n_work_rows = n_rows - cnt;
    return RS_OK;
}

constexpr int RS_POP_MAX = 512;

static int32_t split_popular(rs_knn *h, const int32_t *sorted, const int32_t *len_sorted, int32_t *order, int64_t n_rows,
                             int64_t min_len) {
    cudaStream_t st = h->stream;
    int32_t *d_num;
    RS_TRY(rs_alloc(h, &d_num, 4));
    int32_t cap = RS_POP_MAX;
    if (const char *e = getenv("RS_KNN_POP_MAX")) { cap = atoi(e); cap = cap < 2 ? 2 : (cap > 2048 ? 2048 : cap); }
    pop_count_kernel<<<1, 1, 0, st>>>(len_sorted, h->n_left, min_len, cap, d_num);
    int32_t n_pop = 0;
    RS_CUDA(cudaMemcpyAsync(&n_pop, d_num, 4, cudaMemcpyDeviceToHost, st));
    RS_CUDA(cudaStreamSynchronize(st));
    h->prof.total_launches++;
    if (n_pop < 2) return RS_OK;
    const int32_t nr = h->n_right;
    h->n_pop = n_pop;
    h->pop_ld = (n_pop + 31) / 32 * 32;
    h->pop_u8 = h->rating_class == RS_CLASS_INT8;
    RS_TRY(rs_alloc(h, &h->pop_idx, (size_t)h->n_left));
    RS_TRY(rs_alloc(h, &h->pop_items, (size_t)h->pop_ld));
    RS_TRY(rs_alloc(h, &h->pop_blk, ((size_t)h->n_left + 31) / 32 + 1));
    RS_CUDA(cudaMemsetAsync(h->pop_idx, 0xFF, (size_t)h->n_left * 4, st));
    RS_CUDA(cudaMemsetAsync(h->pop_blk, 0, ((size_t)h->n_left + 31) / 32 + 1, st));
    pop_index_kernel<<<blocks_for(h->pop_ld), T, 0, st>>>(sorted, n_pop, h->pop_ld, h->pop_idx, h->pop_items, h->pop_blk);
    const size_t cell = h->pop_u8 ? 1 : 8;
    RS_TRY(rs_dev_alloc(h, &h->pop_dense, (size_t)nr * h->pop_ld * cell));
    RS_CUDA(cudaMemsetAsync(h->pop_dense, h->pop_u8 ? 0 : 0xFF, (size_t)nr * h->pop_ld * cell, st));
    int64_t *w_cnt, *pos;
    RS_TRY(rs_alloc(h, &w_cnt, (size_t)nr + 1));
    RS_TRY(rs_alloc(h, &h->w_ptr, (size_t)nr + 1));
    RS_TRY(rs_alloc(h, &h->w_col, (size_t)h->nnz));
    RS_TRY(rs_alloc(h, &h->w_dev, (size_t)h->nnz));
    RS_TRY(rs_alloc(h, &pos, (size_t)h->nnz));
    if (h->pop_u8)
        pop_scatter_kernel<uint8_t><<<blocks_for(((int64_t)nr + 1) * 32), T, 0, st>>>(
            h->r_ptr, h->r_col, h->r_val, h->r_dev, nr, h->pop_idx, h->pop_ld, static_cast<uint8_t *>(h->pop_dense), w_cnt);
    else
        pop_scatter_kernel<double><<<blocks_for(((int64_t)nr + 1) * 32), T, 0, st>>>(
            h->r_ptr, h->r_col, h->r_val, h->r_dev, nr, h->pop_idx, h->pop_ld, static_cast<double *>(h->pop_dense), w_cnt);
    size_t need = 0;
    RS_CUDA(cub::DeviceScan::ExclusiveSum(nullptr, need, w_cnt, h->w_ptr, nr + 1, st));
    void *tmp;
    RS_TRY(rs_dev_alloc(h, &tmp, need + 256));
    RS_CUDA(cub::DeviceScan::ExclusiveSum(tmp, need, w_cnt, h->w_ptr, nr + 1, st));
    pop_compact_kernel<<<blocks_for((int64_t)nr * 32), T, 0, st>>>(h->r_ptr, h->r_col, h->r_dev, nr, h->pop_idx, h->w_ptr,
                                                                   h->w_col, h->w_dev, pos);
    pop_remap_l2r_kernel<<<blocks_for(h->nnz), T, 0, st>>>(h->l2r, pos, h->nnz);
    h->prof.total_launches += 5;
    h->row_all = order;
    h->n_all_rows = n_rows;
    int32_t *rest;
    RS_TRY(rs_alloc(h, &rest, (size_t)(n_rows > 0 ? n_rows : 1)));
    h->row_order = rest;
    h->n_work_rows = 0;
    if (n_rows > 0) {
        PopLight light{h->pop_idx};
        size_t need2 = 0;
        RS_CUDA(cub::DeviceSelect::If(nullptr, need2, order, rest, d_num, (int)n_rows, light, st));
        void *tmp2;
        RS_TRY(rs_dev_alloc(h, &tmp2, need2 + 256));
        RS_CUDA(cub::DeviceSelect::If(tmp2, need2, order, rest, d_num, (int)n_rows, light, st));
        int32_t cnt = 0;
        RS_CUDA(cudaMemcpyAsync(&cnt, d_num, 4, cudaMemcpyDeviceToHost, st));
        RS_CUDA(cudaStreamSynchronize(st));
        h->n_work_rows = cnt;
    }
    return RS_OK;
}

int32_t rs_prep_rt(rs_knn *h) {
    cudaStream_t st = h->stream;
    h->n_chunks = (int32_t)(((int64_t)h->n_left + h->stream_jc - 1) / h->stream_jc);
    h->n_pop = 0;
    RS_TRY(rs_alloc(h, &h->r_dev, (size_t)h->nnz));
    RS_TRY(rs_alloc(h, &h->l2r, (size_t)h->nnz));
    RS_TRY(rs_alloc(h, &h->cp, (size_t)h->n_right * ((size_t)h->n_chunks + 1)));
    build_rdev_kernel<<<blocks_for((int64_t)h->n_right * 32), T, 0, st>>>(
        h->r_ptr, h->r_col, h->r_val, h->n_right, h->p.sim, h->pmeans, h->left_bias, h->right_bias, h->global_bias,
        h->r_dev);
    invert_perm_kernel<<<blocks_for(h->nnz), T, 0, st>>>(h->perm_rl, h->nnz, h->perm_tmp);
    compose_l2r_kernel<<<blocks_for(h->nnz), T, 0, st>>>(h->perm_lr, h->perm_tmp, h->nnz, h->l2r);
    h->prof.total_launches += 4;
    auto build_cp = [&]() {
        build_cp_kernel<<<blocks_for((int64_t)h->n_right * 32), T, 0, st>>>(
            h->n_pop ? h->w_ptr : h->r_ptr, h->n_pop ? h->w_col : h->r_col, h->n_right, 0, h->n_chunks, h->stream_jc, h->cp);
    };
    {
        const int64_t rb = h->row_begin, rows = h->row_end - h->row_begin;
        int32_t *len, *len_sorted, *ids, *sorted;
        RS_TRY(rs_alloc(h, &len, (size_t)h->n_left));
        RS_TRY(rs_alloc(h, &len_sorted, (size_t)h->n_left));
        RS_TRY(rs_alloc(h, &ids, (size_t)h->n_left));
        RS_TRY(rs_alloc(h, &sorted, (size_t)h->n_left));
        row_len_kernel<<<blocks_for(h->n_left), T, 0, st>>>(h->l_ptr, h->n_left, len, ids);
        h->prof.total_launches++;
        if (h->p.store == RS_STORE_TOPK) {
            h->row_order = ids;
            h->n_work_rows = -1;
            build_cp();
            RS_CUDA(cudaGetLastError());
            return RS_OK;
        }
        size_t need = 0;
        RS_CUDA(cub::DeviceRadixSort::SortPairsDescending(nullptr, need, len + rb, len_sorted + rb, ids + rb,
                                                          sorted, (int)rows, 0, 32, st));
        void *tmp;
        RS_TRY(rs_dev_alloc(h, &tmp, need));
        RS_CUDA(cub::DeviceRadixSort::SortPairsDescending(tmp, need, len + rb, len_sorted + rb, ids + rb,
                                                          sorted, (int)rows, 0, 32, st));
        const bool full = h->row_begin == 0 && h->row_end == h->n_left;
        int64_t min_len = 8192;
        if (const char *e = getenv("RS_KNN_HEAVY_MIN")) min_len = atoll(e);
        bool pop = full && min_len >= 0;
        if (const char *e = getenv("RS_KNN_POP")) pop = pop && atoi(e) != 0;
        int32_t *order = sorted;
        int64_t n_order = rows;
        if (h->cyc_R > 1) {
            int32_t *owned, *d_num;
            RS_TRY(rs_alloc(h, &owned, (size_t)h->n_left));
            RS_TRY(rs_alloc(h, &d_num, 4));
            size_t need2 = 0;
            CycOwned pred{h->cyc_R, h->cyc_r};
            RS_CUDA(cub::DeviceSelect::If(nullptr, need2, sorted, owned, d_num, (int)h->n_left, pred, st));
            void *tmp2;
            RS_TRY(rs_dev_alloc(h, &tmp2, need2 + 256));
            RS_CUDA(cub::DeviceSelect::If(tmp2, need2, sorted, owned, d_num, (int)h->n_left, pred, st));
            order = owned;
            n_order = h->rows_local;
        }
        h->n_heavy = 0;
        h->row_heavy = nullptr;
        h->row_order = order;
        h->n_work_rows = n_order;
        if (pop) RS_TRY(split_popular(h, sorted, len_sorted, order, n_order, min_len));
        else RS_TRY(split_heavy_rows(h, order, n_order, full));
        build_cp();
    }
    RS_CUDA(cudaGetLastError());
    return RS_OK;
}

int32_t rs_prep_planes(rs_knn *h) {
    cudaStream_t st = h->stream;
    const int32_t kblk = RS_TC_KBLK;
    h->tc_npad = ((int64_t)h->n_left + RS_TC_BM - 1) / RS_TC_BM * RS_TC_BM;
    h->tc_kpad = ((int64_t)h->n_right + RS_TC_KBLK - 1) / RS_TC_KBLK * RS_TC_KBLK;
    size_t bytes = 3 * (size_t)h->tc_npad * (size_t)h->tc_kpad;
    RS_TRY(rs_alloc(h, &h->planes, bytes));
    RS_CUDA(cudaMemsetAsync(h->planes, 0, bytes, st));
    scatter_planes_kernel<<<blocks_for((int64_t)h->n_left * 32), T, 0, st>>>(h->l_ptr, h->l_col, h->l_code,
                                                                            h->n_left, h->tc_npad, h->tc_kpad,
                                                                            kblk, h->planes);
    h->prof.total_launches++;
    RS_CUDA(cudaGetLastError());
    return RS_OK;
}
```

### recommend-sys_b200/csrc/sim_stream.cu

```cuda
#include <cstdlib>
#include <cstring>

#include "common.cuh"

namespace {

constexpr int SW = RS_STREAM_WARPS;

struct StreamArgs {
    const int64_t *l_ptr;
    const int32_t *l_col;
    const double *l_val;
    const int64_t *l2r;
    const int64_t *r_ptr;
    const int32_t *r_col;
    const double *r_dev;
    const int32_t *row_order;
    const int32_t *cp;
    int32_t n_chunks;
    const double *pmeans;
    const double *left_bias, *right_bias;
    double global_bias, shrinkage;
    double *sims;
    int64_t ld_s;
    int32_t n_left;
    int64_t row_begin, row_end;
    int64_t n_rows;
    int cyc_R;
    int symmetric;
    const int32_t *pop_idx;
    unsigned long long *counter;
};

constexpr int G = 8;

template <int SIM, bool SHRINK, int JC>
__device__ __forceinline__ void stream_update(double *acc, int j, double ra, double raa, double rb) {
    if (SIM == RS_SIM_MSD) {
        const double d = ra - rb;
        acc[j] += d * d;
        acc[JC + j] += 1.0;
    } else {
        acc[j] += raa;
        acc[JC + j] += rb * rb;
        acc[2 * JC + j] += ra * rb;
        if (SHRINK) acc[3 * JC + j] += 1.0;
    }
}


struct PopArgs {
    const int32_t *rows;
    int64_t n_rows;
    const int32_t *pop_idx;
    const int32_t *pop_items;
    int32_t n_blk, ld;
    const void *dense;
    int64_t n_first;
    int32_t skip;
};

__device__ __forceinline__ void pop_cp_async16(void *dst, const void *src) {
    asm volatile("cp.async.cg.shared.global [%0], [%1], 16;" ::"r"((uint32_t)__cvta_generic_to_shared(dst)), "l"(src) : "memory");
}
__device__ __forceinline__ void pop_commit() { asm volatile("cp.async.commit_group;" ::: "memory"); }
template <int N> __device__ __forceinline__ void pop_wait() { asm volatile("cp.async.wait_group %0;" ::"n"(N) : "memory"); }

template <int SIM, bool SHRINK, typename DT>
__device__ __forceinline__ void pop_item(const StreamArgs &a, const PopArgs &pa, int64_t item, double *scratch, int lane) {
    constexpr bool U8 = sizeof(DT) == 1;
    double2 *s_a = reinterpret_cast<double2 *>(scratch);
    double *s_rbias = scratch + 64;
    int32_t *s_c = reinterpret_cast<int32_t *>(scratch + 96);
    uint8_t *s_d = reinterpret_cast<uint8_t *>(scratch + 112);
    const DT *__restrict__ dense = static_cast<const DT *>(pa.dense);
    const double nan_v = __longlong_as_double(0x7ff8000000000001ll);
    const int32_t i = pa.rows[item / pa.n_blk];
    const int b = (int)(item % pa.n_blk);
    const int pi = pa.pop_idx[i];
    if (pi >= 0 && 32 * b > pi) return;
    const int col = 32 * b + lane;
    const int32_t hcol = pa.pop_items[col];
    const bool want = hcol >= 0 && (pi < 0 || col < pi);
    double bh = 0.0;
    if (want && SIM == RS_SIM_PEARSON) bh = a.pmeans[hcol];
    if (want && SIM == RS_SIM_PEARSON_BASELINE) bh = a.global_bias + a.left_bias[hcol];
    double ai = 0.0;
    if (SIM == RS_SIM_PEARSON) ai = a.pmeans[i];
    if (SIM == RS_SIM_PEARSON_BASELINE) ai = a.global_bias + a.left_bias[i];
    double acc0 = 0.0, acc1 = 0.0, acc2 = 0.0, acc3 = 0.0;
    const int64_t eb = a.l_ptr[i], ee = a.l_ptr[i + 1];

    auto apply = [&](bool rated, double rb, const double2 aa, double rbias_u) {
        (void)rbias_u;
        if (SIM == RS_SIM_MSD) {
            const double dd = aa.x - rb;
            const double t = dd * dd;
            if (rated) { acc0 += t; acc1 += 1.0; }
        } else {
            const double t1 = rb * rb, t2 = aa.x * rb;
            if (rated) {
                acc0 += aa.y;
                acc1 += t1;
                acc2 += t2;
                if (SHRINK) acc3 += 1.0;
            }
        }
    };

    if (__any_sync(0xffffffffu, want)) {
        int32_t c_0 = 0, c_1 = 0;
        double v_0 = 0.0, v_1 = 0.0;
        if (eb + lane < ee) { c_0 = a.l_col[eb + lane]; v_0 = a.l_val[eb + lane]; }
        if (eb + 32 + lane < ee) { c_1 = a.l_col[eb + 32 + lane]; v_1 = a.l_val[eb + 32 + lane]; }
        auto issue = [&](int32_t c_l, int64_t x0, int buf) {
            if constexpr (U8) {
#pragma unroll
                for (int h2 = 0; h2 < 2; h2++) {
                    const int p = lane + 32 * h2, u = p >> 1;
                    const int32_t c_u = __shfl_sync(0xffffffffu, c_l, u);
                    if (x0 + u < ee)
                        pop_cp_async16(s_d + buf * 1024 + 32 * u + 16 * (p & 1),
                                       reinterpret_cast<const uint8_t *>(dense) + (int64_t)c_u * pa.ld + 32 * b + 16 * (p & 1));
                }
            }
            pop_commit();
        };
        __syncwarp();
        issue(c_0, eb, 0);
        int buf = 0;
        for (int64_t x0 = eb; x0 < ee; x0 += 32, buf ^= 1) {
            const int32_t c = c_0;
            const double v = v_0;
            c_0 = c_1; v_0 = v_1;
            c_1 = 0; v_1 = 0.0;
            if (x0 + 64 + lane < ee) { c_1 = a.l_col[x0 + 64 + lane]; v_1 = a.l_val[x0 + 64 + lane]; }
            double ra = 0.0, rbias = 0.0;
            if (x0 + lane < ee) {
                if (SIM == RS_SIM_PEARSON) ra = v - ai;
                else if (SIM == RS_SIM_PEARSON_BASELINE) { rbias = a.right_bias[c]; const double bb = ai + rbias; ra = v - bb; }
                else ra = v;
            }
            s_a[lane] = make_double2(ra, ra * ra);
            if (SIM == RS_SIM_PEARSON_BASELINE) s_rbias[lane] = rbias;
            if (!U8) s_c[lane] = c;
            issue(c_0, x0 + 32, buf ^ 1);
            pop_wait<1>();
            __syncwarp();
            const int lim = (ee - x0) < 32 ? (int)(ee - x0) : 32;
            if constexpr (U8) {
                const uint8_t *sd = s_d + buf * 1024 + lane;
#pragma unroll 8
                for (int u = 0; u < lim; u++) {
                    const int code = want ? (int)sd[32 * u] : 0;
                    const double y = __hiloint2double(0x43380000, code) - (6755399441055744.0 + (double)RS_INT8_BIAS);
                    const double2 aa = s_a[u];
                    double rb;
                    double rbias_u = 0.0;
                    if (SIM == RS_SIM_PEARSON) rb = y - bh;
                    else if (SIM == RS_SIM_PEARSON_BASELINE) { rbias_u = s_rbias[u]; const double bb = bh + rbias_u; rb = y - bb; }
                    else rb = y;
                    apply(code != 0, rb, aa, rbias_u);
                }
            } else {
                constexpr int PU = 8;
                for (int u0 = 0; u0 < lim; u0 += PU) {
                    double d[PU];
#pragma unroll
                    for (int g = 0; g < PU; g++) {
                        d[g] = nan_v;
                        if (want && u0 + g < lim) d[g] = dense[(int64_t)s_c[u0 + g] * pa.ld + col];
                    }
#pragma unroll
                    for (int g = 0; g < PU; g++) {
                        const int u = (u0 + g) & 31;
                        apply(d[g] == d[g], d[g], s_a[u], 0.0);
                    }
                }
            }
            __syncwarp();
        }
        pop_wait<0>();
    }

    if (hcol >= 0) {
        double *out = a.sims + (a.cyc_R > 1 ? rs_cyc_local(i, a.cyc_R) : (int64_t)(i - a.row_begin)) * a.ld_s;
        if (pi >= 0 && col == pi) {
            out[hcol] = nan_v;
        } else if (want) {
            double s;
            if (SIM == RS_SIM_MSD) s = 1.0 / (acc0 / acc1 + 1.0);
            else s = acc2 / (sqrt(acc0) * sqrt(acc1));
            if (SHRINK) s = (acc3 - 1.0) / (acc3 - 1.0 + a.shrinkage) * s;
            out[hcol] = s;
        }
    }
}

template <int SIM, bool SHRINK, int SYM, int JC, int POP>
__global__ void __launch_bounds__(SW * 32, 4) sim_stream_kernel(StreamArgs a, PopArgs pa) {
    constexpr int NACC = SHRINK ? 4 : 3;
    extern __shared__ double s_acc_all[];
    const int warp = threadIdx.x >> 5, lane = threadIdx.x & 31;
    double *acc = s_acc_all + (size_t)warp * NACC * JC;
    double *s_ra = s_acc_all + (size_t)SW * NACC * JC + warp * 32;
    const int64_t Q = a.n_chunks;
    const int64_t n_items = a.n_rows * Q;
    const double nan_v = __longlong_as_double(0x7ff8000000000001ll);
    const int32_t *__restrict__ r_col = a.r_col;
    const double *__restrict__ r_dev = a.r_dev;

    for (;;) {
        unsigned long long item = 0;
        if (lane == 0) item = atomicAdd(a.counter, 1ull);
        item = __shfl_sync(0xffffffffu, item, 0);
        if (POP) {
            int64_t d = (int64_t)item;
            if (d >= pa.n_first) d = d >= pa.n_first + n_items ? d - n_items : -1;
            if (d >= pa.n_rows * pa.n_blk) break;
            if (pa.skip && ((d >= 0 && d < pa.n_first && (pa.skip & 1)) || (d < 0 && (pa.skip & 2)) || (d >= pa.n_first && (pa.skip & 4)))) continue;
            if (d >= 0) {
                __syncwarp();
                if (POP == 1) pop_item<SIM, SHRINK, uint8_t>(a, pa, d, acc, lane);
                else pop_item<SIM, SHRINK, double>(a, pa, d, acc, lane);
                __syncwarp();
                continue;
            }
            item -= (unsigned long long)pa.n_first;
        } else if ((int64_t)item >= n_items) break;
        const int64_t q = (int64_t)item % Q;
        const int32_t i = a.row_order[(int64_t)item / Q];
        const int j0 = (int)(q * JC);
        if (SYM == 1 && j0 + JC <= i) continue;
        if (SYM == 2 && j0 > i) continue;

        for (int x = lane; x < NACC * JC; x += 32) acc[x] = 0.0;

        double ai = 0.0;
        if (SIM == RS_SIM_PEARSON) ai = a.pmeans[i];
        if (SIM == RS_SIM_PEARSON_BASELINE) ai = a.global_bias + a.left_bias[i];

        const int64_t eb = a.l_ptr[i], ee = a.l_ptr[i + 1];
        for (int64_t x0 = eb; x0 < ee; x0 += 32) {
            const int64_t e = x0 + lane;
            double ra = 0.0;
            uint32_t lo = 0, self = 0xffffffffu;
            int n = 0;
            if (e < ee) {
                const int32_t c = a.l_col[e];
                const double v = a.l_val[e];
                if (SIM == RS_SIM_PEARSON) ra = v - ai;
                else if (SIM == RS_SIM_PEARSON_BASELINE) { const double bb = ai + a.right_bias[c]; ra = v - bb; }
                else ra = v;
                const int64_t rp = a.r_ptr[c];
                const int32_t *cpc = a.cp + (int64_t)c * (Q + 1) + q;
                int64_t lo64 = rp + cpc[0];
                int64_t hi = rp + cpc[1];
                const int64_t self64 = a.l2r[e];
                if (SYM == 1) { if (self64 + 1 > lo64) lo64 = self64 + 1; }
                else if (SYM == 2) { if (self64 < hi) hi = self64; }
                else self = (uint32_t)self64;
                n = hi > lo64 ? (int)(hi - lo64) : 0;
                lo = (uint32_t)lo64;
            }
            __syncwarp();
            s_ra[lane] = ra;
            __syncwarp();
            const int lim = (ee - x0) < 32 ? (int)(ee - x0) : 32;
            for (int u0 = 0; u0 < lim; u0 += G) {
                int jj[G], nn[G];
                double rbv[G];
#pragma unroll
                for (int g = 0; g < G; g++) {
                    const int u = u0 + g;
                    nn[g] = __shfl_sync(0xffffffffu, n, u);
                    const uint32_t lo_u = __shfl_sync(0xffffffffu, lo, u);
                    uint32_t self_u = 0xffffffffu;
                    if (!SYM) self_u = __shfl_sync(0xffffffffu, self, u);
                    jj[g] = -1;
                    rbv[g] = 0.0;
                    if (lane < nn[g]) {
                        const uint32_t idx = lo_u + (uint32_t)lane;
                        if (SYM || idx != self_u) {
                            jj[g] = r_col[idx] - j0;
                            rbv[g] = r_dev[idx];
                        }
                    }
                }
#pragma unroll
                for (int g = 0; g < G; g++) {
                    if (nn[g] == 0) continue;
                    const double ra_u = s_ra[u0 + g];
                    const double raa_u = ra_u * ra_u;
                    if (jj[g] >= 0) stream_update<SIM, SHRINK, JC>(acc, jj[g], ra_u, raa_u, rbv[g]);
                    if (nn[g] > 32) {
                        const uint32_t lo_u = __shfl_sync(0xffffffffu, lo, u0 + g);
                        uint32_t self_u = 0xffffffffu;
                        if (!SYM) self_u = __shfl_sync(0xffffffffu, self, u0 + g);
                        for (int t = lane + 32; t < nn[g]; t += 32) {
                            const uint32_t idx = lo_u + (uint32_t)t;
                            if (!SYM && idx == self_u) continue;
                            stream_update<SIM, SHRINK, JC>(acc, r_col[idx] - j0, ra_u, raa_u, r_dev[idx]);
                        }
                    }
                    __syncwarp();
                }
            }
        }
        __syncwarp();

        double *out = a.sims + (a.cyc_R > 1 ? rs_cyc_local(i, a.cyc_R) : (int64_t)(i - a.row_begin)) * a.ld_s + j0;
        for (int j = lane; j < JC; j += 32) {
            const int64_t col = (int64_t)j0 + j;
            if (col >= a.n_left) break;
            if (SYM == 1 && col < i) continue;
            if (SYM == 2 && col > i) break;
            if (a.pop_idx && a.pop_idx[col] >= 0) continue;
            double s;
            if (SIM == RS_SIM_MSD) s = 1.0 / (acc[j] / acc[JC + j] + 1.0);
            else s = acc[2 * JC + j] / (sqrt(acc[j]) * sqrt(acc[JC + j]));
            if (SHRINK) {
                const double cn = acc[3 * JC + j];
                s = (cn - 1.0) / (cn - 1.0 + a.shrinkage) * s;
            }
            if (col == (int64_t)i) s = nan_v;
            out[j] = s;
        }
        __syncwarp();
    }
}



constexpr int HV_CONS = 4, HV_PROD = 8, HV_WARPS = HV_CONS + HV_PROD;
constexpr int HV_SLOTS = 32;
constexpr int HV_DEPTH = 3;
constexpr int HV_JC = 256;

struct HeavyArgs {
    const int32_t *rows;
    int32_t n_rows;
    unsigned long long *counter;
};

__device__ __forceinline__ uint32_t hv_smem_u32(const void *p) { return (uint32_t)__cvta_generic_to_shared(p); }
__device__ __forceinline__ void hv_cp_async4(void *dst, const void *src) {
    asm volatile("cp.async.ca.shared.global [%0], [%1], 4;" ::"r"(hv_smem_u32(dst)), "l"(src) : "memory");
}
__device__ __forceinline__ void hv_cp_async8(void *dst, const void *src) {
    asm volatile("cp.async.ca.shared.global [%0], [%1], 8;" ::"r"(hv_smem_u32(dst)), "l"(src) : "memory");
}
__device__ __forceinline__ void hv_commit() { asm volatile("cp.async.commit_group;" ::: "memory"); }
template <int N> __device__ __forceinline__ void hv_wait() { asm volatile("cp.async.wait_group %0;" ::"n"(N) : "memory"); }

template <int SIM, bool SHRINK>
__global__ void __launch_bounds__(HV_WARPS * 32, 1) sim_stream_heavy_kernel(StreamArgs a, HeavyArgs hv) {
    constexpr int NACC = SHRINK ? 4 : 3;
    extern __shared__ double hv_smem[];
    double *acc = hv_smem;
    double *s_rb = acc + NACC * HV_JC;
    int32_t *s_jc = reinterpret_cast<int32_t *>(s_rb + HV_SLOTS * HV_JC);
    double *s_ra = reinterpret_cast<double *>(s_jc + HV_SLOTS * HV_JC);
    int32_t *s_n = reinterpret_cast<int32_t *>(s_ra + HV_SLOTS);
    volatile int32_t *s_ready = s_n + HV_SLOTS;
    volatile int32_t *s_consumed = s_ready + HV_SLOTS;
    volatile long long *s_item = reinterpret_cast<volatile long long *>(s_consumed + HV_CONS);
    const int warp = threadIdx.x >> 5, lane = threadIdx.x & 31;
    const int64_t Q = a.n_chunks;
    const int64_t n_items = (int64_t)hv.n_rows * Q;
    const double nan_v = __longlong_as_double(0x7ff8000000000001ll);

    for (;;) {
        __syncthreads();
        if (threadIdx.x == 0) *s_item = (long long)atomicAdd(hv.counter, 1ull);
        if (threadIdx.x < HV_SLOTS) s_ready[threadIdx.x] = 0;
        if (threadIdx.x < HV_CONS) s_consumed[threadIdx.x] = 0;
        __syncthreads();
        const int64_t item = *s_item;
        if (item >= n_items) break;
        const int64_t q = item % Q;
        const int32_t i = hv.rows[item / Q];
        const int j0 = (int)(q * HV_JC);
        if (a.symmetric == 1 && j0 + HV_JC <= i) continue;
        if (a.symmetric == 2 && j0 > i) continue;
        const bool diag_chunk = (i >= j0 && i < j0 + HV_JC);
        const int64_t eb = a.l_ptr[i], ee = a.l_ptr[i + 1];
        const int n_ent = (int)(ee - eb);

        if (warp < HV_CONS) {
            const int cw = warp;
#pragma unroll
            for (int z = 0; z < NACC; z++)
                for (int x = lane; x < 64; x += 32) acc[z * HV_JC + 64 * cw + x] = 0.0;
            __syncwarp();
            for (int e = 0; e < n_ent; e++) {
                const int slot = e % HV_SLOTS;
                int word;
                while (((word = s_ready[slot]) >> 9) != e + 1) {}
                __syncwarp();
                const int n = word & 511;
                if (n > 0) {
                    const double ra = s_ra[slot];
                    const double raa = ra * ra;
                    const double *rbs = s_rb + slot * HV_JC;
                    const int32_t *jcs = s_jc + slot * HV_JC;
                    auto apply = [&](int j, double rb) {
                        if (SIM == RS_SIM_MSD) {
                            const double d = ra - rb;
                            acc[j] += d * d;
                            acc[HV_JC + j] += 1.0;
                        } else {
                            acc[j] += raa;
                            acc[HV_JC + j] += rb * rb;
                            acc[2 * HV_JC + j] += ra * rb;
                            if (SHRINK) acc[3 * HV_JC + j] += 1.0;
                        }
                    };
                    if (n <= 64) {
                        int jv[2];
                        double rbv[2];
#pragma unroll
                        for (int u = 0; u < 2; u++) {
                            const int t = lane + 32 * u;
                            jv[u] = t < n ? jcs[t] - j0 : -1;
                            rbv[u] = t < n ? rbs[t] : 0.0;
                        }
#pragma unroll
                        for (int u = 0; u < 2; u++) if (jv[u] >= 0 && (jv[u] >> 6) == cw) apply(jv[u], rbv[u]);
                    } else {
                        int jv[8];
                        double rbv[8];
#pragma unroll
                        for (int u = 0; u < 8; u++) {
                            const int t = lane + 32 * u;
                            jv[u] = t < n ? jcs[t] - j0 : -1;
                            rbv[u] = t < n ? rbs[t] : 0.0;
                        }
#pragma unroll
                        for (int u = 0; u < 8; u++) {
                            const bool mine = jv[u] >= 0 && (jv[u] >> 6) == cw;
                            if (!__any_sync(0xffffffffu, mine)) continue;
                            if (mine) apply(jv[u], rbv[u]);
                        }
                    }
                }
                __syncwarp();
                if (lane == 0) s_consumed[cw] = e + 1;
            }
            __syncwarp();
            double *out = a.sims + (a.cyc_R > 1 ? rs_cyc_local(i, a.cyc_R) : (int64_t)(i - a.row_begin)) * a.ld_s + j0;
            for (int j = 64 * cw + lane; j < 64 * cw + 64; j += 32) {
                const int64_t col = (int64_t)j0 + j;
                if (col >= a.n_left) break;
                if (a.symmetric == 1 && col < i) continue;
                if (a.symmetric == 2 && col > i) break;
                double s;
                if (SIM == RS_SIM_MSD) s = 1.0 / (acc[j] / acc[HV_JC + j] + 1.0);
                else s = acc[2 * HV_JC + j] / (sqrt(acc[j]) * sqrt(acc[HV_JC + j]));
                if (SHRINK) {
                    const double cn = acc[3 * HV_JC + j];
                    s = (cn - 1.0) / (cn - 1.0 + a.shrinkage) * s;
                }
                if (col == (int64_t)i) s = nan_v;
                out[j] = s;
            }
        } else {
            const int p = warp - HV_CONS;
            double ai = 0.0;
            if (SIM == RS_SIM_PEARSON) ai = a.pmeans[i];
            if (SIM == RS_SIM_PEARSON_BASELINE) ai = a.global_bias + a.left_bias[i];
            auto ent_of = [&](int k) { return p + k * HV_PROD; };
            int issued = 0, published = 0;
            auto publish = [&](int k) {
                __syncwarp();
                __threadfence_block();
                if (lane == 0) { const int e = ent_of(k); s_ready[e % HV_SLOTS] = ((e + 1) << 9) | s_n[e % HV_SLOTS]; }
            };
            const int my_total = n_ent > p ? (n_ent - p + HV_PROD - 1) / HV_PROD : 0;
            for (int k0 = 0; k0 < my_total; k0 += 32) {
                const int k_l = k0 + lane;
                double ra_l = 0.0;
                uint32_t lo_l = 0;
                int n_l = 0;
                if (k_l < my_total) {
                    const int64_t e = eb + ent_of(k_l);
                    const int32_t c = a.l_col[e];
                    const double v = a.l_val[e];
                    if (SIM == RS_SIM_PEARSON) ra_l = v - ai;
                    else if (SIM == RS_SIM_PEARSON_BASELINE) { const double bb = ai + a.right_bias[c]; ra_l = v - bb; }
                    else ra_l = v;
                    const int64_t rp = a.r_ptr[c];
                    const int32_t *cpc = a.cp + (int64_t)c * (Q + 1) + q;
                    int64_t lo64 = rp + cpc[0];
                    int64_t hi = rp + cpc[1];
                    if (diag_chunk) {
                        const int64_t self64 = a.l2r[e];
                        if (a.symmetric == 1) { if (self64 + 1 > lo64) lo64 = self64 + 1; }
                        else { if (self64 < hi) hi = self64; }
                    }
                    n_l = hi > lo64 ? (int)(hi - lo64) : 0;
                    lo_l = (uint32_t)lo64;
                }
                const int lim = my_total - k0 < 32 ? my_total - k0 : 32;
                for (int u = 0; u < lim; u++) {
                    const int k = k0 + u;
                    const int e = ent_of(k);
                    const int slot = e % HV_SLOTS;
                    const double ra_u = __shfl_sync(0xffffffffu, ra_l, u);
                    const uint32_t lo_u = __shfl_sync(0xffffffffu, lo_l, u);
                    const int n_u = __shfl_sync(0xffffffffu, n_l, u);
                    for (bool first = true;; first = false) {
                        int done = s_consumed[0];
#pragma unroll
                        for (int z = 1; z < HV_CONS; z++) { const int d = s_consumed[z]; done = d < done ? d : done; }
                        if (done >= e - HV_SLOTS + 1) break;
                        if (first) {
                            hv_wait<0>();
                            while (published < issued) { publish(published); published++; }
                        }
                        __nanosleep(40);
                    }
                    __syncwarp();
                    for (int t = lane; t < n_u; t += 32) {
                        hv_cp_async4(s_jc + slot * HV_JC + t, a.r_col + lo_u + t);
                        hv_cp_async8(s_rb + slot * HV_JC + t, a.r_dev + lo_u + t);
                    }
                    if (lane == 0) { s_ra[slot] = ra_u; s_n[slot] = n_u; }
                    hv_commit();
                    issued++;
                    if (issued - published > HV_DEPTH) {
                        hv_wait<HV_DEPTH>();
                        publish(published);
                        published++;
                    }
                }
            }
            hv_wait<0>();
            while (published < issued) { publish(published); published++; }
        }
    }
}

__device__ __forceinline__ bool pop_owns(int64_t r, int64_t c, int pr, int pc, int lower) {
    if (pc >= 0 && pr < 0) return true;
    if (pr >= 0 && pc < 0) return false;
    if (pr >= 0) return pc < pr;
    return lower ? c < r : c > r;
}

__global__ void symmetrize_kernel(double *__restrict__ s, int64_t ld, int32_t n, int lower) {
    __shared__ double tile[32][33];
    int64_t bi = blockIdx.y, bj = blockIdx.x;
    if (bj > bi) return;
    if (lower) { const int64_t t = bi; bi = bj; bj = t; }
    const int64_t r0 = bi * 32, c0 = bj * 32;
    for (int y = threadIdx.y; y < 32; y += blockDim.y) {
        int64_t sr = c0 + y, sc = r0 + threadIdx.x;
        tile[y][threadIdx.x] = (sr < n && sc < n) ? s[sr * ld + sc] : 0.0;
    }
    __syncthreads();
    for (int y = threadIdx.y; y < 32; y += blockDim.y) {
        int64_t r = r0 + y, c = c0 + threadIdx.x;
        if (r < n && c < n && (lower ? c > r : c < r)) s[r * ld + c] = tile[threadIdx.x][y];
    }
}

struct MirrorArgs {
    double *self;
    const double *peer[RS_MAX_PEERS];
    int64_t ld;
    int32_t n;
    int32_t count, index, lower;
};
__global__ void mirror_kernel(MirrorArgs a) {
    __shared__ double tile[32][33];
    const int64_t bI = blockIdx.y;
    const int64_t gI = bI * a.count + a.index, gJ = blockIdx.x;
    if (a.lower ? gJ < gI : gJ > gI) return;
    const double *src = a.peer[gJ % a.count];
    const int64_t sJ = (gJ / a.count) * RS_CYC_B;
    for (int y = threadIdx.y; y < 32; y += blockDim.y) {
        const int64_t sr = gJ * 32 + y, sc = gI * 32 + threadIdx.x;
        tile[y][threadIdx.x] = (sr < a.n && sc < a.n) ? src[(sJ + y) * a.ld + sc] : 0.0;
    }
    __syncthreads();
    for (int y = threadIdx.y; y < 32; y += blockDim.y) {
        const int64_t r = gI * 32 + y, c = gJ * 32 + threadIdx.x;
        if (r < a.n && c < a.n && (a.lower ? c > r : c < r)) a.self[(bI * 32 + y) * a.ld + c] = tile[threadIdx.x][y];
    }
}

__global__ void symmetrize_pop_kernel(double *__restrict__ s, int64_t ld, int32_t n, int lower,
                                      const int32_t *__restrict__ pop_idx, const uint8_t *__restrict__ pop_blk) {
    __shared__ double ta[32][33], tb[32][33];
    const int64_t bi = blockIdx.y, bj = blockIdx.x;
    if (bj > bi) return;
    if (!(pop_blk[bi] | pop_blk[bj])) {
        const int64_t di = lower ? bj : bi, dj = lower ? bi : bj;
        const int64_t r0 = di * 32, c0 = dj * 32;
        for (int y = threadIdx.y; y < 32; y += blockDim.y) {
            const int64_t sr = c0 + y, sc = r0 + threadIdx.x;
            ta[y][threadIdx.x] = (sr < n && sc < n) ? s[sr * ld + sc] : 0.0;
        }
        __syncthreads();
        for (int y = threadIdx.y; y < 32; y += blockDim.y) {
            const int64_t r = r0 + y, c = c0 + threadIdx.x;
            if (r < n && c < n && (lower ? c > r : c < r)) s[r * ld + c] = ta[threadIdx.x][y];
        }
        return;
    }
    const int64_t r0 = bi * 32, c0 = bj * 32;
    for (int y = threadIdx.y; y < 32; y += blockDim.y) {
        const int64_t ar = r0 + y, ac = c0 + threadIdx.x, br = c0 + y, bc = r0 + threadIdx.x;
        ta[y][threadIdx.x] = (ar < n && ac < n) ? s[ar * ld + ac] : 0.0;
        tb[y][threadIdx.x] = (br < n && bc < n) ? s[br * ld + bc] : 0.0;
    }
    __syncthreads();
    for (int y = threadIdx.y; y < 32; y += blockDim.y) {
        int64_t r = r0 + y, c = c0 + threadIdx.x;
        if (r < n && c < n && r != c && !pop_owns(r, c, pop_idx[r], pop_idx[c], lower)) s[r * ld + c] = tb[threadIdx.x][y];
        if (bi == bj) continue;
        r = c0 + y; c = r0 + threadIdx.x;
        if (r < n && c < n && !pop_owns(r, c, pop_idx[r], pop_idx[c], lower)) s[r * ld + c] = ta[threadIdx.x][y];
    }
}

__global__ void mirror_pop_kernel(MirrorArgs a, const int32_t *__restrict__ pop_idx) {
    __shared__ double tile[32][33];
    const int64_t bI = blockIdx.y;
    const int64_t gI = bI * a.count + a.index, gJ = blockIdx.x;
    bool need[4];
    bool any = false;
#pragma unroll
    for (int k = 0; k < 4; k++) {
        const int y = threadIdx.y + 8 * k;
        const int64_t r = gI * 32 + y, c = gJ * 32 + threadIdx.x;
        need[k] = r < a.n && c < a.n && r != c && !pop_owns(r, c, pop_idx[r], pop_idx[c], a.lower);
        any = any || need[k];
    }
    if (!__syncthreads_or(any)) return;
    const double *src = a.peer[gJ % a.count];
    const int64_t sJ = (gJ / a.count) * RS_CYC_B;
    for (int y = threadIdx.y; y < 32; y += blockDim.y) {
        const int64_t sr = gJ * 32 + y, sc = gI * 32 + threadIdx.x;
        tile[y][threadIdx.x] = (sr < a.n && sc < a.n) ? src[(sJ + y) * a.ld + sc] : 0.0;
    }
    __syncthreads();
#pragma unroll
    for (int k = 0; k < 4; k++) {
        const int y = threadIdx.y + 8 * k;
        if (need[k]) a.self[(bI * 32 + y) * a.ld + gJ * 32 + threadIdx.x] = tile[threadIdx.x][y];
    }
}

}

template <int SIM, bool SHRINK, int SYM, int JC, int POP>
static int32_t launch_stream_pop(rs_knn *h, const StreamArgs &s, const PopArgs &pa, int grid) {
    const int smem = SW * ((SHRINK ? 4 : 3) * JC + 32) * (int)sizeof(double);
    auto kern = sim_stream_kernel<SIM, SHRINK, SYM, JC, POP>;
    RS_CUDA(cudaFuncSetAttribute(kern, cudaFuncAttributeMaxDynamicSharedMemorySize, smem));
    kern<<<grid, SW * 32, smem, h->stream>>>(s, pa);
    return RS_OK;
}
template <int SIM, bool SHRINK, int SYM, int JC>
static int32_t launch_stream_jc(rs_knn *h, const StreamArgs &s, const PopArgs &pa, int grid) {
    if (SYM != 0 && s.pop_idx) {
        if (h->pop_u8) return launch_stream_pop<SIM, SHRINK, SYM ? SYM : 1, JC, 1>(h, s, pa, grid);
        return launch_stream_pop<SIM, SHRINK, SYM ? SYM : 1, JC, 2>(h, s, pa, grid);
    }
    return launch_stream_pop<SIM, SHRINK, SYM, JC, 0>(h, s, pa, grid);
}
template <int SIM, bool SHRINK, int SYM>
static int32_t launch_stream_sym(rs_knn *h, const StreamArgs &s, const PopArgs &pa, int grid) {
    if (h->stream_jc == 128) return launch_stream_jc<SIM, SHRINK, SYM, 128>(h, s, pa, grid);
    return launch_stream_jc<SIM, SHRINK, SYM, 256>(h, s, pa, grid);
}
template <int SIM, bool SHRINK>
static int32_t launch_stream(rs_knn *h, const StreamArgs &s, const PopArgs &pa, int grid) {
    if (h->nnz >= (int64_t)0xffffffffll) {
        rs_set_error("stream path indexes the ratings with 32 bits (nnz=%lld)", (long long)h->nnz);
        return RS_ERR_UNSUPPORTED;
    }
    if (s.symmetric == 2) return launch_stream_sym<SIM, SHRINK, 2>(h, s, pa, grid);
    return s.symmetric ? launch_stream_sym<SIM, SHRINK, 1>(h, s, pa, grid) : launch_stream_sym<SIM, SHRINK, 0>(h, s, pa, grid);
}

template <int SIM, bool SHRINK>
static int32_t launch_heavy(rs_knn *h, const StreamArgs &a, const HeavyArgs &hv) {
    constexpr int NACC = SHRINK ? 4 : 3;
    const int smem = (NACC * HV_JC + HV_SLOTS * HV_JC) * 8 + HV_SLOTS * HV_JC * 4 + HV_SLOTS * 8 + HV_SLOTS * 4 * 2 + HV_CONS * 4 + 64;
    auto kern = sim_stream_heavy_kernel<SIM, SHRINK>;
    RS_CUDA(cudaFuncSetAttribute(kern, cudaFuncAttributeMaxDynamicSharedMemorySize, smem));
    int sms = 148;
    cudaDeviceGetAttribute(&sms, cudaDevAttrMultiProcessorCount, h->device);
    int64_t grid = (int64_t)hv.n_rows * a.n_chunks;
    if (grid > sms) grid = sms;
    kern<<<(unsigned)grid, HV_WARPS * 32, smem, h->aux_stream>>>(a, hv);
    h->prof.total_launches += 1;
    return RS_OK;
}

static int32_t rs_heavy_rows_launch(rs_knn *h, const StreamArgs &a, const HeavyArgs &hv) {
    switch (h->p.sim) {
    case RS_SIM_COSINE: return launch_heavy<RS_SIM_COSINE, false>(h, a, hv);
    case RS_SIM_MSD: return launch_heavy<RS_SIM_MSD, false>(h, a, hv);
    case RS_SIM_PEARSON: return launch_heavy<RS_SIM_PEARSON, false>(h, a, hv);
    case RS_SIM_PEARSON_BASELINE:
        return h->p.shrinkage > 0.0 ? launch_heavy<RS_SIM_PEARSON_BASELINE, true>(h, a, hv)
                                    : launch_heavy<RS_SIM_PEARSON_BASELINE, false>(h, a, hv);
    default: rs_set_error("unknown similarity %d", h->p.sim); return RS_ERR_INVALID;
    }
}

int32_t rs_sim_stream_launch(rs_knn *h) {
    StreamArgs a{};
    a.l_ptr = h->l_ptr; a.l_col = h->l_col; a.l_val = h->l_val; a.l2r = h->l2r;
    a.r_ptr = h->r_ptr; a.r_col = h->r_col; a.r_dev = h->r_dev; a.cp = h->cp; a.n_chunks = h->n_chunks;
    const bool cyc = h->cyc_R > 1;
    a.row_order = h->n_work_rows >= 0 ? h->row_order : h->row_order + h->row_begin;
    a.n_rows = h->n_work_rows >= 0 ? h->n_work_rows : h->row_end - h->row_begin;
    a.cyc_R = h->cyc_R;
    a.pmeans = h->pmeans; a.left_bias = h->left_bias; a.right_bias = h->right_bias;
    a.global_bias = h->global_bias; a.shrinkage = h->p.shrinkage;
    a.sims = h->sims; a.ld_s = h->ld_s; a.n_left = h->n_left;
    a.row_begin = h->row_begin; a.row_end = h->row_end;
    a.symmetric = h->force_sym ? 1 : ((h->row_begin == 0 && h->row_end == h->n_left) || cyc) ? (h->stream_lower ? 2 : 1) : 0;
    a.counter = reinterpret_cast<unsigned long long *>(h->d_flags + 2);
    RS_CUDA(cudaMemsetAsync(a.counter, 0, 8, h->stream));
    const bool pop = h->n_pop > 0;
    PopArgs pa{};
    if (pop) {
        if (a.symmetric == 0 || h->force_sym) {
            rs_set_error("popular columns were split off, but this Fit does not compute a triangle of the full matrix");
            return RS_ERR_INVALID;
        }
        a.r_ptr = h->w_ptr; a.r_col = h->w_col; a.r_dev = h->w_dev; a.pop_idx = h->pop_idx;
        pa.rows = h->row_all; pa.n_rows = h->n_all_rows;
        pa.pop_idx = h->pop_idx; pa.pop_items = h->pop_items;
        pa.n_blk = h->pop_ld / 32; pa.ld = h->pop_ld;
        pa.dense = h->pop_dense;
        pa.n_first = (h->n_all_rows - a.n_rows) * pa.n_blk;
        if (const char *e = getenv("RS_KNN_STREAM_SKIP")) pa.skip = atoi(e);
    }
    const bool heavy = !pop && h->n_heavy > 0 && a.symmetric != 0 && !h->force_sym && h->stream_jc == HV_JC;
    if (heavy) {
        HeavyArgs hv{};
        hv.rows = h->row_heavy; hv.n_rows = h->n_heavy;
        hv.counter = reinterpret_cast<unsigned long long *>(h->d_flags + 12);
        RS_CUDA(cudaMemsetAsync(hv.counter, 0, 8, h->stream));
        RS_CUDA(cudaEventRecord(h->ev_fork, h->stream));
        RS_CUDA(cudaStreamWaitEvent(h->aux_stream, h->ev_fork, 0));
        RS_TRY(rs_heavy_rows_launch(h, a, hv));
        RS_CUDA(cudaEventRecord(h->ev_join, h->aux_stream));
    }
    if (a.n_rows <= 0 && !(pop && pa.n_rows > 0)) {
        if (heavy) RS_CUDA(cudaStreamWaitEvent(h->stream, h->ev_join, 0));
        return RS_OK;
    }
    int sms = 148;
    cudaDeviceGetAttribute(&sms, cudaDevAttrMultiProcessorCount, h->device);
    const int64_t items = a.n_rows * (int64_t)h->n_chunks + (pop ? pa.n_rows * pa.n_blk : 0);
    int64_t grid = (int64_t)sms * 4;
    if (grid > (items + SW - 1) / SW) grid = (items + SW - 1) / SW;
    switch (h->p.sim) {
    case RS_SIM_COSINE: RS_TRY((launch_stream<RS_SIM_COSINE, false>(h, a, pa, (int)grid))); break;
    case RS_SIM_MSD: RS_TRY((launch_stream<RS_SIM_MSD, false>(h, a, pa, (int)grid))); break;
    case RS_SIM_PEARSON: RS_TRY((launch_stream<RS_SIM_PEARSON, false>(h, a, pa, (int)grid))); break;
    case RS_SIM_PEARSON_BASELINE:
        if (h->p.shrinkage > 0.0) RS_TRY((launch_stream<RS_SIM_PEARSON_BASELINE, true>(h, a, pa, (int)grid)));
        else RS_TRY((launch_stream<RS_SIM_PEARSON_BASELINE, false>(h, a, pa, (int)grid)));
        break;
    default: rs_set_error("unknown similarity %d", h->p.sim); return RS_ERR_INVALID;
    }
    if (heavy) RS_CUDA(cudaStreamWaitEvent(h->stream, h->ev_join, 0));
    h->prof.sim_launches++;
    h->prof.total_launches++;
    RS_CUDA(cudaGetLastError());
    return RS_OK;
}

int32_t rs_mirror_launch(rs_knn *h) {
    MirrorArgs a{};
    a.self = h->sims;
    for (int q = 0; q < h->cyc_R; q++) a.peer[q] = h->peer_sims[q];
    a.peer[h->cyc_r] = h->sims;
    a.ld = h->ld_s; a.n = h->n_left; a.count = h->cyc_R; a.index = h->cyc_r; a.lower = h->stream_lower ? 1 : 0;
    const int64_t nblk = ((int64_t)h->n_left + RS_CYC_B - 1) / RS_CYC_B;
    const int64_t own = (nblk - h->cyc_r + h->cyc_R - 1) / h->cyc_R;
    if (own <= 0) return RS_OK;
    dim3 grid((unsigned)nblk, (unsigned)own), block(32, 8);
    if (h->n_pop > 0) mirror_pop_kernel<<<grid, block, 0, h->stream>>>(a, h->pop_idx);
    else mirror_kernel<<<grid, block, 0, h->stream>>>(a);
    h->prof.total_launches++;
    RS_CUDA(cudaGetLastError());
    return RS_OK;
}

int32_t rs_symmetrize_launch(rs_knn *h) {
    if (h->cyc_R > 1) return RS_OK;
    if (!(h->row_begin == 0 && h->row_end == h->n_left)) return RS_OK;
    const unsigned t = (unsigned)((h->n_left + 31) / 32);
    dim3 grid(t, t), block(32, 8);
    if (h->n_pop > 0) symmetrize_pop_kernel<<<grid, block, 0, h->stream>>>(h->sims, h->ld_s, h->n_left, h->stream_lower ? 1 : 0, h->pop_idx, h->pop_blk);
    else symmetrize_kernel<<<grid, block, 0, h->stream>>>(h->sims, h->ld_s, h->n_left, h->stream_lower ? 1 : 0);
    h->prof.total_launches++;
    RS_CUDA(cudaGetLastError());
    return RS_OK;
}
```

Baseline: 6.008 billion.

## Relabel light items by popularity rank for the streaming similarity walk

```diff
diff --git a/recommend-sys_b200/csrc/api.cu b/recommend-sys_b200/csrc/api.cu
--- a/recommend-sys_b200/csrc/api.cu
+++ b/recommend-sys_b200/csrc/api.cu
@@ -49,9 +49,8 @@
     h->row_heavy = nullptr;
     h->n_heavy = 0;
     h->n_pop = h->pop_ld = 0;
-    h->pop_idx = h->pop_items = nullptr;
+    h->rank = h->lab_row = h->pop_items = nullptr;
     h->pop_dense = nullptr;
-    h->pop_blk = nullptr;
     h->w_ptr = nullptr;
     h->w_col = nullptr;
     h->w_dev = nullptr;
diff --git a/recommend-sys_b200/csrc/common.cuh b/recommend-sys_b200/csrc/common.cuh
--- a/recommend-sys_b200/csrc/common.cuh
+++ b/recommend-sys_b200/csrc/common.cuh
@@ -134,9 +134,9 @@
     int32_t n_heavy = 0;
     int32_t n_pop = 0, pop_ld = 0;
     bool pop_u8 = false;
-    int32_t *pop_idx = nullptr;
+    int32_t *rank = nullptr;
+    int32_t *lab_row = nullptr;
     int32_t *pop_items = nullptr;
-    uint8_t *pop_blk = nullptr;
     void *pop_dense = nullptr;
     int64_t *w_ptr = nullptr;
     int32_t *w_col = nullptr;
diff --git a/recommend-sys_b200/csrc/prep.cu b/recommend-sys_b200/csrc/prep.cu
--- a/recommend-sys_b200/csrc/prep.cu
+++ b/recommend-sys_b200/csrc/prep.cu
@@ -217,64 +217,62 @@
     }
     *out = lo < cap ? lo : cap;
 }
-__global__ void pop_index_kernel(const int32_t *__restrict__ sorted, int32_t n_pop, int32_t pop_ld,
-                                 int32_t *__restrict__ pop_idx, int32_t *__restrict__ pop_items,
-                                 uint8_t *__restrict__ pop_blk) {
+__global__ void pop_items_kernel(const int32_t *__restrict__ sorted, int32_t n_pop, int32_t pop_ld,
+                                 int32_t *__restrict__ pop_items) {
     const int32_t p = blockIdx.x * blockDim.x + threadIdx.x;
-    if (p >= pop_ld) return;
-    if (p < n_pop) { const int32_t i = sorted[p]; pop_idx[i] = p; pop_items[p] = i; pop_blk[i >> 5] = 1; }
-    else pop_items[p] = -1;
+    if (p < pop_ld) pop_items[p] = p < n_pop ? sorted[p] : -1;
 }
 template <typename DT>
 __global__ void pop_scatter_kernel(const int64_t *__restrict__ r_ptr, const int32_t *__restrict__ r_col,
                                    const double *__restrict__ r_val, const double *__restrict__ r_dev,
-                                   int32_t n_right, const int32_t *__restrict__ pop_idx, int32_t pop_ld,
-                                   DT *__restrict__ dense, int64_t *__restrict__ w_cnt) {
-    const int32_t c = (int32_t)(((int64_t)blockIdx.x * blockDim.x + threadIdx.x) >> 5);
-    const int lane = threadIdx.x & 31;
-    if (c > n_right) return;
-    if (c == n_right) { if (lane == 0) w_cnt[c] = 0; return; }
-    int32_t light = 0;
-    for (int64_t x = r_ptr[c] + lane; x < r_ptr[c + 1]; x += 32) {
-        const int32_t p = pop_idx[r_col[x]];
-        if (p < 0) { light++; continue; }
-        if (sizeof(DT) == 1) dense[(int64_t)c * pop_ld + p] = (DT)((int)r_val[x] + RS_INT8_BIAS);
-        else dense[(int64_t)c * pop_ld + p] = (DT)r_dev[x];
-    }
-#pragma unroll
-    for (int o = 16; o > 0; o >>= 1) light += __shfl_xor_sync(0xffffffffu, light, o);
-    if (lane == 0) w_cnt[c] = light;
-}
-__global__ void pop_compact_kernel(const int64_t *__restrict__ r_ptr, const int32_t *__restrict__ r_col,
-                                   const double *__restrict__ r_dev, int32_t n_right,
-                                   const int32_t *__restrict__ pop_idx, const int64_t *__restrict__ w_ptr,
-                                   int32_t *__restrict__ w_col, double *__restrict__ w_dev, int64_t *__restrict__ pos) {
+                                   int32_t n_right, const int32_t *__restrict__ rank, int32_t n_pop, int32_t pop_ld,
+                                   DT *__restrict__ dense) {
     const int32_t c = (int32_t)(((int64_t)blockIdx.x * blockDim.x + threadIdx.x) >> 5);
     const int lane = threadIdx.x & 31;
     if (c >= n_right) return;
-    const int64_t b = r_ptr[c], e = r_ptr[c + 1];
-    int64_t out = w_ptr[c];
-    for (int64_t x0 = b; x0 < e; x0 += 32) {
-        const int64_t x = x0 + lane;
-        int32_t j = -1;
-        bool keep = false;
-        if (x < e) { j = r_col[x]; keep = pop_idx[j] < 0; }
-        const unsigned m = __ballot_sync(0xffffffffu, keep);
-        if (x < e) {
-            const int64_t o = out + __popc(m & ((1u << lane) - 1u));
-            if (keep) { w_col[o] = j; w_dev[o] = r_dev[x]; pos[x] = o; }
-            else pos[x] = -1;
-        }
-        out += __popc(m);
-    }
-}
-__global__ void pop_remap_l2r_kernel(int64_t *__restrict__ l2r, const int64_t *__restrict__ pos, int64_t n) {
-    const int64_t e = (int64_t)blockIdx.x * blockDim.x + threadIdx.x;
-    if (e < n) l2r[e] = pos[l2r[e]];
+    for (int64_t x = r_ptr[c] + lane; x < r_ptr[c + 1]; x += 32) {
+        const int32_t p = rank[r_col[x]];
+        if (p >= n_pop) continue;
+        if (sizeof(DT) == 1) dense[(int64_t)c * pop_ld + p] = (DT)((int)r_val[x] + RS_INT8_BIAS);
+        else dense[(int64_t)c * pop_ld + p] = (DT)r_dev[x];
+    }
+}
+__global__ void walk_seq_kernel(const int32_t *__restrict__ sorted, int32_t n_left, int32_t n_pop,
+                                const int64_t *__restrict__ l_ptr, const int32_t *__restrict__ l_col,
+                                const int64_t *__restrict__ w_off, int32_t *__restrict__ key, int32_t *__restrict__ ent,
+                                int32_t *__restrict__ ent_lab, int64_t *__restrict__ l2r) {
+    const int32_t p = (int32_t)(((int64_t)blockIdx.x * blockDim.x + threadIdx.x) >> 5);
+    const int lane = threadIdx.x & 31;
+    if (p >= n_left) return;
+    const int32_t i = sorted[p];
+    const int64_t b = l_ptr[i], e = l_ptr[i + 1];
+    if (p < n_pop) {
+        for (int64_t x = b + lane; x < e; x += 32) l2r[x] = -1;
+        return;
+    }
+    const int32_t lab = p - n_pop;
+    const int64_t o = w_off[lab] - b;
+#pragma unroll 4
+    for (int64_t x = b + lane; x < e; x += 32) {
+        key[o + x] = l_col[x];
+        ent[o + x] = (int32_t)x;
+        ent_lab[x] = lab;
+    }
+}
+__global__ void walk_gather_kernel(const int32_t *__restrict__ ent, const int32_t *__restrict__ ent_lab,
+                                   const double *__restrict__ r_dev, int64_t n, int32_t *__restrict__ w_col,
+                                   double *__restrict__ w_dev, int64_t *__restrict__ l2r) {
+    const int64_t o = (int64_t)blockIdx.x * blockDim.x + threadIdx.x;
+    if (o >= n) return;
+    const int32_t x = ent[o];
+    w_col[o] = ent_lab[x];
+    w_dev[o] = r_dev[l2r[x]];
+    l2r[x] = o;
 }
 struct PopLight {
-    const int32_t *pop_idx;
-    __host__ __device__ bool operator()(const int32_t &i) const { return pop_idx[i] < 0; }
+    const int32_t *rank;
+    int32_t n_pop;
+    __host__ __device__ bool operator()(const int32_t &i) const { return rank[i] >= n_pop; }
 };
 
 
@@ -344,12 +342,12 @@
     if ((threadIdx.x & 31) == 0 && acc) atomicAdd(out, acc);
 }
 
-__global__ void incidence_kernel(const int64_t *__restrict__ l_ptr, int32_t nl, int32_t jc,
-                                 unsigned long long *out) {
+__global__ void incidence_kernel(const int64_t *__restrict__ l_ptr, const int32_t *__restrict__ len, int32_t nl,
+                                 int32_t jc, unsigned long long *out) {
     unsigned long long up = 0, lo = 0;
     const long long q_all = (nl + jc - 1) / jc;
     for (int64_t i = blockIdx.x * (int64_t)blockDim.x + threadIdx.x; i < nl; i += (int64_t)gridDim.x * blockDim.x) {
-        const unsigned long long d = (unsigned long long)(l_ptr[i + 1] - l_ptr[i]);
+        const unsigned long long d = (unsigned long long)(len ? (int64_t)len[i] : l_ptr[i + 1] - l_ptr[i]);
         const long long q = i / jc;
         up += d * (unsigned long long)(q_all - q);
         lo += d * (unsigned long long)(q + 1);
@@ -372,6 +370,11 @@
 #pragma unroll
     for (int o = 16; o > 0; o >>= 1) s += __shfl_xor_sync(0xffffffffu, s, o);
     if (lane == 0) out[c] = s / (double)(r_ptr[c + 1] - r_ptr[c]);
+}
+
+static void pick_triangle(rs_knn *h) {
+    h->stream_lower = h->inc_lower < h->inc_upper;
+    if (const char *e = getenv("RS_KNN_STREAM_TRI")) h->stream_lower = !strcmp(e, "lower");
 }
 
 static int32_t rs_stream_jc(int32_t n_left) {
@@ -428,7 +431,7 @@
     gather_keys_kernel<<<blocks_for(nnz), T, 0, st>>>(d_left, perm_r, nnz, keys_a);
     RS_SORT_PAIRS(keys_a, keys_b, perm_r, perm_lr, nnz, lb);
     ptr_from_sorted_kernel<<<blocks_for(nnz + 1), T, 0, st>>>(keys_b, nnz, nl, h->l_ptr);
-    incidence_kernel<<<148, T, 0, st>>>(h->l_ptr, nl, h->stream_jc, reinterpret_cast<unsigned long long *>(h->d_flags + 8));
+    incidence_kernel<<<148, T, 0, st>>>(h->l_ptr, nullptr, nl, h->stream_jc, reinterpret_cast<unsigned long long *>(h->d_flags + 8));
     h->prof.total_launches += 4;
     gather_keys_kernel<<<blocks_for(nnz), T, 0, st>>>(d_right, perm_lr, nnz, keys_a);
     RS_SORT_PAIRS(keys_a, keys_b, perm_lr, perm_rl, nnz, rb);
@@ -498,8 +501,7 @@
     { unsigned long long t; memcpy(&t, fl8 + 6, 8); h->triples = (double)t; }
     h->max_right_len = fl8[15];
     { unsigned long long t[2]; memcpy(t, fl8 + 8, 16); h->inc_upper = (double)t[0]; h->inc_lower = (double)t[1]; }
-    h->stream_lower = h->inc_lower < h->inc_upper;
-    if (const char *e = getenv("RS_KNN_STREAM_TRI")) h->stream_lower = !strcmp(e, "lower");
+    pick_triangle(h);
     if (flags & FLAG_DUP) {
         rs_set_error("duplicate (left,right) rating pairs are not supported (the reference's merge-join "
                      "double-counts them)");
@@ -560,58 +562,85 @@
     RS_CUDA(cudaStreamSynchronize(st));
     h->prof.total_launches++;
     if (n_pop < 2) return RS_OK;
-    const int32_t nr = h->n_right;
+    const int32_t nr = h->n_right, nl = h->n_left, n_walk = nl - n_pop;
     h->n_pop = n_pop;
     h->pop_ld = (n_pop + 31) / 32 * 32;
     h->pop_u8 = h->rating_class == RS_CLASS_INT8;
-    RS_TRY(rs_alloc(h, &h->pop_idx, (size_t)h->n_left));
+    h->lab_row = const_cast<int32_t *>(sorted) + n_pop;
+    RS_TRY(rs_alloc(h, &h->rank, (size_t)nl));
     RS_TRY(rs_alloc(h, &h->pop_items, (size_t)h->pop_ld));
-    RS_TRY(rs_alloc(h, &h->pop_blk, ((size_t)h->n_left + 31) / 32 + 1));
-    RS_CUDA(cudaMemsetAsync(h->pop_idx, 0xFF, (size_t)h->n_left * 4, st));
-    RS_CUDA(cudaMemsetAsync(h->pop_blk, 0, ((size_t)h->n_left + 31) / 32 + 1, st));
-    pop_index_kernel<<<blocks_for(h->pop_ld), T, 0, st>>>(sorted, n_pop, h->pop_ld, h->pop_idx, h->pop_items, h->pop_blk);
+    invert_perm_kernel<<<blocks_for(nl), T, 0, st>>>(sorted, nl, h->rank);
+    pop_items_kernel<<<blocks_for(h->pop_ld), T, 0, st>>>(sorted, n_pop, h->pop_ld, h->pop_items);
     const size_t cell = h->pop_u8 ? 1 : 8;
     RS_TRY(rs_dev_alloc(h, &h->pop_dense, (size_t)nr * h->pop_ld * cell));
     RS_CUDA(cudaMemsetAsync(h->pop_dense, h->pop_u8 ? 0 : 0xFF, (size_t)nr * h->pop_ld * cell, st));
-    int64_t *w_cnt, *pos;
-    RS_TRY(rs_alloc(h, &w_cnt, (size_t)nr + 1));
-    RS_TRY(rs_alloc(h, &h->w_ptr, (size_t)nr + 1));
-    RS_TRY(rs_alloc(h, &h->w_col, (size_t)h->nnz));
-    RS_TRY(rs_alloc(h, &h->w_dev, (size_t)h->nnz));
-    RS_TRY(rs_alloc(h, &pos, (size_t)h->nnz));
     if (h->pop_u8)
-        pop_scatter_kernel<uint8_t><<<blocks_for(((int64_t)nr + 1) * 32), T, 0, st>>>(
-            h->r_ptr, h->r_col, h->r_val, h->r_dev, nr, h->pop_idx, h->pop_ld, static_cast<uint8_t *>(h->pop_dense), w_cnt);
+        pop_scatter_kernel<uint8_t><<<blocks_for((int64_t)nr * 32), T, 0, st>>>(
+            h->r_ptr, h->r_col, h->r_val, h->r_dev, nr, h->rank, n_pop, h->pop_ld, static_cast<uint8_t *>(h->pop_dense));
     else
-        pop_scatter_kernel<double><<<blocks_for(((int64_t)nr + 1) * 32), T, 0, st>>>(
-            h->r_ptr, h->r_col, h->r_val, h->r_dev, nr, h->pop_idx, h->pop_ld, static_cast<double *>(h->pop_dense), w_cnt);
-    size_t need = 0;
-    RS_CUDA(cub::DeviceScan::ExclusiveSum(nullptr, need, w_cnt, h->w_ptr, nr + 1, st));
-    void *tmp;
-    RS_TRY(rs_dev_alloc(h, &tmp, need + 256));
-    RS_CUDA(cub::DeviceScan::ExclusiveSum(tmp, need, w_cnt, h->w_ptr, nr + 1, st));
-    pop_compact_kernel<<<blocks_for((int64_t)nr * 32), T, 0, st>>>(h->r_ptr, h->r_col, h->r_dev, nr, h->pop_idx, h->w_ptr,
-                                                                   h->w_col, h->w_dev, pos);
-    pop_remap_l2r_kernel<<<blocks_for(h->nnz), T, 0, st>>>(h->l2r, pos, h->nnz);
-    h->prof.total_launches += 5;
+        pop_scatter_kernel<double><<<blocks_for((int64_t)nr * 32), T, 0, st>>>(
+            h->r_ptr, h->r_col, h->r_val, h->r_dev, nr, h->rank, n_pop, h->pop_ld, static_cast<double *>(h->pop_dense));
+    h->prof.total_launches += 3;
+    int64_t *w_off;
+    unsigned long long *d_inc;
+    RS_TRY(rs_alloc(h, &w_off, (size_t)n_walk + 1));
+    RS_TRY(rs_alloc(h, &d_inc, 2));
+    RS_CUDA(cudaMemsetAsync(w_off, 0, 8, st));
+    RS_CUDA(cudaMemsetAsync(d_inc, 0, 16, st));
+    if (n_walk > 0) {
+        size_t need = 0;
+        RS_CUDA(cub::DeviceScan::InclusiveSum(nullptr, need, len_sorted + n_pop, w_off + 1, n_walk, st));
+        void *tmp;
+        RS_TRY(rs_dev_alloc(h, &tmp, need + 256));
+        RS_CUDA(cub::DeviceScan::InclusiveSum(tmp, need, len_sorted + n_pop, w_off + 1, n_walk, st));
+    }
+    incidence_kernel<<<148, T, 0, st>>>(nullptr, len_sorted + n_pop, n_walk, h->stream_jc, d_inc);
+    h->prof.total_launches++;
     h->row_all = order;
     h->n_all_rows = n_rows;
     int32_t *rest;
     RS_TRY(rs_alloc(h, &rest, (size_t)(n_rows > 0 ? n_rows : 1)));
     h->row_order = rest;
-    h->n_work_rows = 0;
+    int32_t cnt = 0;
     if (n_rows > 0) {
-        PopLight light{h->pop_idx};
+        PopLight light{h->rank, n_pop};
         size_t need2 = 0;
         RS_CUDA(cub::DeviceSelect::If(nullptr, need2, order, rest, d_num, (int)n_rows, light, st));
         void *tmp2;
         RS_TRY(rs_dev_alloc(h, &tmp2, need2 + 256));
         RS_CUDA(cub::DeviceSelect::If(tmp2, need2, order, rest, d_num, (int)n_rows, light, st));
-        int32_t cnt = 0;
         RS_CUDA(cudaMemcpyAsync(&cnt, d_num, 4, cudaMemcpyDeviceToHost, st));
-        RS_CUDA(cudaStreamSynchronize(st));
-        h->n_work_rows = cnt;
-    }
+    }
+    int64_t nnz_w = 0;
+    unsigned long long inc[2] = {0, 0};
+    RS_CUDA(cudaMemcpyAsync(&nnz_w, w_off + n_walk, 8, cudaMemcpyDeviceToHost, st));
+    RS_CUDA(cudaMemcpyAsync(inc, d_inc, 16, cudaMemcpyDeviceToHost, st));
+    RS_CUDA(cudaStreamSynchronize(st));
+    h->n_work_rows = cnt;
+    h->inc_upper = (double)inc[0];
+    h->inc_lower = (double)inc[1];
+    pick_triangle(h);
+    h->n_chunks = (int32_t)(((int64_t)n_walk + h->stream_jc - 1) / h->stream_jc);
+    int32_t *key, *ent, *key_s, *ent_s, *ent_lab;
+    RS_TRY(rs_alloc(h, &h->w_ptr, (size_t)nr + 1));
+    RS_TRY(rs_alloc(h, &h->w_col, (size_t)nnz_w));
+    RS_TRY(rs_alloc(h, &h->w_dev, (size_t)nnz_w));
+    RS_TRY(rs_alloc(h, &key, (size_t)nnz_w));
+    RS_TRY(rs_alloc(h, &ent, (size_t)nnz_w));
+    RS_TRY(rs_alloc(h, &key_s, (size_t)nnz_w));
+    RS_TRY(rs_alloc(h, &ent_s, (size_t)nnz_w));
+    RS_TRY(rs_alloc(h, &ent_lab, (size_t)h->nnz));
+    walk_seq_kernel<<<blocks_for((int64_t)nl * 32), T, 0, st>>>(sorted, nl, n_pop, h->l_ptr, h->l_col, w_off, key, ent,
+                                                                ent_lab, h->l2r);
+    h->prof.total_launches++;
+    if (nnz_w > 0) {
+        SortTmp tmp;
+        RS_SORT_PAIRS(key, key_s, ent, ent_s, nnz_w, bits_for(nr));
+        walk_gather_kernel<<<blocks_for(nnz_w), T, 0, st>>>(ent_s, ent_lab, h->r_dev, nnz_w, h->w_col, h->w_dev, h->l2r);
+        h->prof.total_launches++;
+    }
+    ptr_from_sorted_kernel<<<blocks_for(nnz_w + 1), T, 0, st>>>(key_s, nnz_w, nr, h->w_ptr);
+    h->prof.total_launches++;
     return RS_OK;
 }
 
diff --git a/recommend-sys_b200/csrc/sim_stream.cu b/recommend-sys_b200/csrc/sim_stream.cu
--- a/recommend-sys_b200/csrc/sim_stream.cu
+++ b/recommend-sys_b200/csrc/sim_stream.cu
@@ -28,7 +28,9 @@
     int64_t n_rows;
     int cyc_R;
     int symmetric;
-    const int32_t *pop_idx;
+    const int32_t *rank;
+    const int32_t *lab_row;
+    int32_t n_pop;
     unsigned long long *counter;
 };
 
@@ -52,7 +54,8 @@
 struct PopArgs {
     const int32_t *rows;
     int64_t n_rows;
-    const int32_t *pop_idx;
+    const int32_t *rank;
+    int32_t n_pop;
     const int32_t *pop_items;
     int32_t n_blk, ld;
     const void *dense;
@@ -77,7 +80,7 @@
     const double nan_v = __longlong_as_double(0x7ff8000000000001ll);
     const int32_t i = pa.rows[item / pa.n_blk];
     const int b = (int)(item % pa.n_blk);
-    const int pi = pa.pop_idx[i];
+    const int pi = pa.rank[i] < pa.n_pop ? pa.rank[i] : -1;
     if (pi >= 0 && 32 * b > pi) return;
     const int col = 32 * b + lane;
     const int32_t hcol = pa.pop_items[col];
@@ -230,9 +233,10 @@
         } else if ((int64_t)item >= n_items) break;
         const int64_t q = (int64_t)item % Q;
         const int32_t i = a.row_order[(int64_t)item / Q];
+        const int32_t li = POP ? a.rank[i] - a.n_pop : i;
         const int j0 = (int)(q * JC);
-        if (SYM == 1 && j0 + JC <= i) continue;
-        if (SYM == 2 && j0 > i) continue;
+        if (SYM == 1 && j0 + JC <= li) continue;
+        if (SYM == 2 && j0 > li) continue;
 
         for (int x = lane; x < NACC * JC; x += 32) acc[x] = 0.0;
 
@@ -309,13 +313,8 @@
         }
         __syncwarp();
 
-        double *out = a.sims + (a.cyc_R > 1 ? rs_cyc_local(i, a.cyc_R) : (int64_t)(i - a.row_begin)) * a.ld_s + j0;
-        for (int j = lane; j < JC; j += 32) {
-            const int64_t col = (int64_t)j0 + j;
-            if (col >= a.n_left) break;
-            if (SYM == 1 && col < i) continue;
-            if (SYM == 2 && col > i) break;
-            if (a.pop_idx && a.pop_idx[col] >= 0) continue;
+        double *out = a.sims + (a.cyc_R > 1 ? rs_cyc_local(i, a.cyc_R) : (int64_t)(i - a.row_begin)) * a.ld_s + (POP ? 0 : j0);
+        auto emit = [&](int j, int64_t col) {
             double s;
             if (SIM == RS_SIM_MSD) s = 1.0 / (acc[j] / acc[JC + j] + 1.0);
             else s = acc[2 * JC + j] / (sqrt(acc[j]) * sqrt(acc[JC + j]));
@@ -323,8 +322,23 @@
                 const double cn = acc[3 * JC + j];
                 s = (cn - 1.0) / (cn - 1.0 + a.shrinkage) * s;
             }
-            if (col == (int64_t)i) s = nan_v;
-            out[j] = s;
+            if (col == (int64_t)li) s = nan_v;
+            out[POP ? a.lab_row[col] : j] = s;
+        };
+        if (POP) {
+            for (int j = lane; j < JC; j += 32) {
+                const int64_t col = (int64_t)j0 + j;
+                if (col >= a.n_left - a.n_pop) break;
+                if (SYM == 1 && col < li) continue;
+                if (SYM == 2 && col > li) break;
+                emit(j, col);
+            }
+        } else {
+            int j_end = a.n_left - j0;
+            if (SYM == 2 && li - j0 + 1 < j_end) j_end = li - j0 + 1;
+            if (j_end > JC) j_end = JC;
+            const int j_beg = SYM == 1 && li > j0 ? li - j0 : 0;
+            for (int j = j_beg + lane; j < j_end; j += 32) emit(j, j0 + j);
         }
         __syncwarp();
     }
@@ -541,11 +555,9 @@
     }
 }
 
-__device__ __forceinline__ bool pop_owns(int64_t r, int64_t c, int pr, int pc, int lower) {
-    if (pc >= 0 && pr < 0) return true;
-    if (pr >= 0 && pc < 0) return false;
-    if (pr >= 0) return pc < pr;
-    return lower ? c < r : c > r;
+__device__ __forceinline__ bool pop_owns(int32_t rr, int32_t rc, int32_t n_pop, int lower) {
+    if (!lower && rr >= n_pop && rc >= n_pop) return rr < rc;
+    return rr > rc;
 }
 
 __global__ void symmetrize_kernel(double *__restrict__ s, int64_t ld, int32_t n, int lower) {
@@ -591,25 +603,16 @@
 }
 
 __global__ void symmetrize_pop_kernel(double *__restrict__ s, int64_t ld, int32_t n, int lower,
-                                      const int32_t *__restrict__ pop_idx, const uint8_t *__restrict__ pop_blk) {
+                                      const int32_t *__restrict__ rank, int32_t n_pop) {
     __shared__ double ta[32][33], tb[32][33];
+    __shared__ int32_t rk_a[32], rk_b[32];
     const int64_t bi = blockIdx.y, bj = blockIdx.x;
     if (bj > bi) return;
-    if (!(pop_blk[bi] | pop_blk[bj])) {
-        const int64_t di = lower ? bj : bi, dj = lower ? bi : bj;
-        const int64_t r0 = di * 32, c0 = dj * 32;
-        for (int y = threadIdx.y; y < 32; y += blockDim.y) {
-            const int64_t sr = c0 + y, sc = r0 + threadIdx.x;
-            ta[y][threadIdx.x] = (sr < n && sc < n) ? s[sr * ld + sc] : 0.0;
-        }
-        __syncthreads();
-        for (int y = threadIdx.y; y < 32; y += blockDim.y) {
-            const int64_t r = r0 + y, c = c0 + threadIdx.x;
-            if (r < n && c < n && (lower ? c > r : c < r)) s[r * ld + c] = ta[threadIdx.x][y];
-        }
-        return;
-    }
     const int64_t r0 = bi * 32, c0 = bj * 32;
+    if (threadIdx.y == 0) {
+        rk_a[threadIdx.x] = r0 + threadIdx.x < n ? rank[r0 + threadIdx.x] : 0;
+        rk_b[threadIdx.x] = c0 + threadIdx.x < n ? rank[c0 + threadIdx.x] : 0;
+    }
     for (int y = threadIdx.y; y < 32; y += blockDim.y) {
         const int64_t ar = r0 + y, ac = c0 + threadIdx.x, br = c0 + y, bc = r0 + threadIdx.x;
         ta[y][threadIdx.x] = (ar < n && ac < n) ? s[ar * ld + ac] : 0.0;
@@ -618,14 +621,14 @@
     __syncthreads();
     for (int y = threadIdx.y; y < 32; y += blockDim.y) {
         int64_t r = r0 + y, c = c0 + threadIdx.x;
-        if (r < n && c < n && r != c && !pop_owns(r, c, pop_idx[r], pop_idx[c], lower)) s[r * ld + c] = tb[threadIdx.x][y];
+        if (r < n && c < n && r != c && !pop_owns(rk_a[y], rk_b[threadIdx.x], n_pop, lower)) s[r * ld + c] = tb[threadIdx.x][y];
         if (bi == bj) continue;
         r = c0 + y; c = r0 + threadIdx.x;
-        if (r < n && c < n && !pop_owns(r, c, pop_idx[r], pop_idx[c], lower)) s[r * ld + c] = ta[threadIdx.x][y];
-    }
-}
-
-__global__ void mirror_pop_kernel(MirrorArgs a, const int32_t *__restrict__ pop_idx) {
+        if (r < n && c < n && !pop_owns(rk_b[y], rk_a[threadIdx.x], n_pop, lower)) s[r * ld + c] = ta[threadIdx.x][y];
+    }
+}
+
+__global__ void mirror_pop_kernel(MirrorArgs a, const int32_t *__restrict__ rank, int32_t n_pop) {
     __shared__ double tile[32][33];
     const int64_t bI = blockIdx.y;
     const int64_t gI = bI * a.count + a.index, gJ = blockIdx.x;
@@ -635,7 +638,7 @@
     for (int k = 0; k < 4; k++) {
         const int y = threadIdx.y + 8 * k;
         const int64_t r = gI * 32 + y, c = gJ * 32 + threadIdx.x;
-        need[k] = r < a.n && c < a.n && r != c && !pop_owns(r, c, pop_idx[r], pop_idx[c], a.lower);
+        need[k] = r < a.n && c < a.n && r != c && !pop_owns(rank[r], rank[c], n_pop, a.lower);
         any = any || need[k];
     }
     if (!__syncthreads_or(any)) return;
@@ -665,7 +668,7 @@
 }
 template <int SIM, bool SHRINK, int SYM, int JC>
 static int32_t launch_stream_jc(rs_knn *h, const StreamArgs &s, const PopArgs &pa, int grid) {
-    if (SYM != 0 && s.pop_idx) {
+    if (SYM != 0 && s.rank) {
         if (h->pop_u8) return launch_stream_pop<SIM, SHRINK, SYM ? SYM : 1, JC, 1>(h, s, pa, grid);
         return launch_stream_pop<SIM, SHRINK, SYM ? SYM : 1, JC, 2>(h, s, pa, grid);
     }
@@ -735,9 +738,10 @@
             rs_set_error("popular columns were split off, but this Fit does not compute a triangle of the full matrix");
             return RS_ERR_INVALID;
         }
-        a.r_ptr = h->w_ptr; a.r_col = h->w_col; a.r_dev = h->w_dev; a.pop_idx = h->pop_idx;
+        a.r_ptr = h->w_ptr; a.r_col = h->w_col; a.r_dev = h->w_dev;
+        a.rank = h->rank; a.lab_row = h->lab_row; a.n_pop = h->n_pop;
         pa.rows = h->row_all; pa.n_rows = h->n_all_rows;
-        pa.pop_idx = h->pop_idx; pa.pop_items = h->pop_items;
+        pa.rank = h->rank; pa.n_pop = h->n_pop; pa.pop_items = h->pop_items;
         pa.n_blk = h->pop_ld / 32; pa.ld = h->pop_ld;
         pa.dense = h->pop_dense;
         pa.n_first = (h->n_all_rows - a.n_rows) * pa.n_blk;
@@ -790,7 +794,7 @@
     const int64_t own = (nblk - h->cyc_r + h->cyc_R - 1) / h->cyc_R;
     if (own <= 0) return RS_OK;
     dim3 grid((unsigned)nblk, (unsigned)own), block(32, 8);
-    if (h->n_pop > 0) mirror_pop_kernel<<<grid, block, 0, h->stream>>>(a, h->pop_idx);
+    if (h->n_pop > 0) mirror_pop_kernel<<<grid, block, 0, h->stream>>>(a, h->rank, h->n_pop);
     else mirror_kernel<<<grid, block, 0, h->stream>>>(a);
     h->prof.total_launches++;
     RS_CUDA(cudaGetLastError());
@@ -802,7 +806,7 @@
     if (!(h->row_begin == 0 && h->row_end == h->n_left)) return RS_OK;
     const unsigned t = (unsigned)((h->n_left + 31) / 32);
     dim3 grid(t, t), block(32, 8);
-    if (h->n_pop > 0) symmetrize_pop_kernel<<<grid, block, 0, h->stream>>>(h->sims, h->ld_s, h->n_left, h->stream_lower ? 1 : 0, h->pop_idx, h->pop_blk);
+    if (h->n_pop > 0) symmetrize_pop_kernel<<<grid, block, 0, h->stream>>>(h->sims, h->ld_s, h->n_left, h->stream_lower ? 1 : 0, h->rank, h->n_pop);
     else symmetrize_kernel<<<grid, block, 0, h->stream>>>(h->sims, h->ld_s, h->n_left, h->stream_lower ? 1 : 0);
     h->prof.total_launches++;
     RS_CUDA(cudaGetLastError());
```

Result: faster. 6.578 billion (median of 6 runs) (+9.5%).
